# lucidrains/transfusion-pytorch

Measured on AMD Instinct MI355X. Metric: train samples/sec, dim512 d8 seq1024 text+latent, higher is better.
Workload: dtype bf16; 1 GPU; BASELINE config 2: Transfusion dim=512 depth=8 heads=8 dim_head=64 num_text_tokens=256 dim_latent=384; per-GPU batch 64 x seq 1024 (32 x [24 text tokens + (4,384) latent] per sample); step = pack + fwd + bwd + clip(0.5) + Adam(3e-4) (one GPU: no gradient exchange); global_batch=64, seq_len=1024, parallelism=dp1

## Files before the change

include/tfx.h:

```cpp
#ifndef TFX_H
#define TFX_H
#include <stdint.h>
#ifdef __cplusplus
extern "C" {
#endif

#ifndef TFX_BF16_DEFINED
typedef uint16_t tfx_bf16;
#endif

enum { TFX_EPI_BF16 = 0, TFX_EPI_F32 = 1, TFX_EPI_SILU = 2, TFX_EPI_RESID = 3, TFX_EPI_GEGLU = 4, TFX_EPI_GEGLU_BWD = 5, TFX_EPI_QKV_NORM_ROPE = 6 };

typedef struct {
  const tfx_bf16* A; int32_t lda;
  const tfx_bf16* A2; int32_t lda2; int32_t K1;
  const tfx_bf16* B; int32_t ldb;
  int32_t M, N, K;
  int32_t epi;
  void* C; int32_t ldc;
  void* C2; int32_t ldc2;
  const float* bias;
  const tfx_bf16* R; int32_t ldr; int32_t resid_mapped;
  const int32_t* rowmap;
  const int32_t* a_rowmap;
// ... 163 lines not shown
int tfx_attnres_finish(const tfx_attnres_src* src_dev, int32_t n, int32_t d, void* stream);
int tfx_adaln_pre_post_bwd(const tfx_adaln_pre_args* pre, const tfx_adaln_post_args* post, void* stream);

typedef struct {
  int32_t T, d;
  const tfx_bf16* x; tfx_bf16* y; const float* gamma;
  const tfx_bf16* dy; tfx_bf16* dx; float* dgamma;
} tfx_rmsnorm_args;
int tfx_rmsnorm_fwd(const tfx_rmsnorm_args* a, void* stream);
int tfx_rmsnorm_bwd(const tfx_rmsnorm_args* a, void* stream);

typedef struct {
  int32_t T, d;
  const int32_t* text_ids; const int32_t* tok_inst;
  const tfx_bf16* table;
  tfx_bf16* x;
  const tfx_bf16* dx; float* dtable;
} tfx_embed_args;
int tfx_embed_fwd(const tfx_embed_args* a, void* stream);
int tfx_embed_bwd(const tfx_embed_args* a, void* stream);

typedef struct {
  int32_t R, dl;
  const float* x; const float* eps;
  const int32_t* row_inst; const float* inst_time;
  tfx_bf16* xt; int32_t ld_xt;
  float* flow;
} tfx_noise_mix_args;
int tfx_noise_mix(const tfx_noise_mix_args* a, void* stream);

typedef struct { int32_t I, half; const float* times; const float* w; tfx_bf16* out; int32_t ld; } tfx_fourier_args;
int tfx_fourier(const tfx_fourier_args* a, void* stream);

typedef struct {
  int32_t T, V; const float* logits; int32_t ld;
  const int32_t* labels;
  float grad_scale;
  tfx_bf16* dlogits; int32_t ld_d;
  float* acc;
} tfx_ce_args;
int tfx_ce_fwd_bwd(const tfx_ce_args* a, void* stream);

typedef struct {
  int32_t R, dl; const float* pred; int32_t ld_pred; const float* flow;
  float grad_scale;
  tfx_bf16* dpred; int32_t ld_d;
  float* acc;
  int32_t accumulate;
  const int32_t* row_inst; const float* inst_time; float clean_eps;
  const float* recon_w; const int32_t* recon_inst; const float* recon_time; int32_t recon_mode;
} tfx_mse_args;
int tfx_mse_fwd_bwd(const tfx_mse_args* a, void* stream);
typedef struct {
  int32_t T, d; const tfx_bf16* pred; int32_t ld_pred; const tfx_bf16* target; int32_t ld_target;
  int32_t n_pad, n_valid;
  float grad_scale;
  tfx_bf16* dpred; int32_t ld_d;
  float* acc;
} tfx_cosine_args;
int tfx_cosine_fwd_bwd(const tfx_cosine_args* a, void* stream);
int tfx_output_to_flow(float* pred, const float* x, const float* eps, const int32_t* row_inst, const float* inst_time,
                       int32_t R, int32_t dl, float clean_eps, void* stream);

int tfx_sample_tokens(const float* logits, int32_t ld, int32_t B, int32_t V, float temperature, float min_p, const float* uniforms,
                      const int32_t* active, int32_t* out_ids, void* stream);
int tfx_sample_tokens_range(const float* logits, int32_t ld, int32_t B, int32_t V, int32_t V_draw, float temperature, float min_p, const float* uniforms,
                            const int32_t* active, int32_t* out_ids, void* stream);
int tfx_ode_axpy(const float* y, const float* f_cond, const float* f_uncond, float cfg_scale, float a, float* out, int64_t n, void* stream);
int tfx_ode_stage(const float* y, const float* ym, const float* ctl, int32_t B, int32_t Lc, int32_t dmax, float* x, int32_t H, int32_t Lq, int32_t dl,
                  const int32_t* rows0, void* stream);
int tfx_ode_update(float* y, float* ym, const float* ctl, int32_t B, int32_t Lc, int32_t dmax, const float* pred, int32_t H, int32_t Lq, int32_t dl,
                   float cfg_scale, const float* sel, const int32_t* rows0, void* stream);
enum { TFX_ODE_MAX_STAGES = 4 };
int tfx_ode_rk_axpy(const float* y, const float* k, int64_t k_stride, int32_t nk, float w0, float w1, float w2, float w3, const float* f_cond,
                    const float* f_uncond, float cfg_scale, float* k_out, float* out, int64_t n, void* stream);
int tfx_ode_rk_stage(const float* y, const float* k, const float* ctl, int32_t B, int32_t Lc, int32_t dmax, float* x, int32_t H, int32_t Lq, int32_t dl,
                     const int32_t* rows0, void* stream);
int tfx_ode_rk_update(float* y, float* k, const float* ctl, int32_t B, int32_t Lc, int32_t dmax, const float* pred, int32_t H, int32_t Lq, int32_t dl,
                      float cfg_scale, const float* sel, const int32_t* rows0, void* stream);

typedef struct { const float* src; int32_t ld_src, Rs, Cs; const int32_t* rowmap; tfx_bf16* dst; int32_t ld_dst, Rd, Cd; } tfx_cast_args;
int tfx_cast_rows(const tfx_cast_args* a, void* stream);
int tfx_cast_rows_t(const tfx_cast_args* a, void* stream);
typedef struct { const float* src; int32_t ld_src, Rs, Cs; const int32_t* rowmap; tfx_bf16* dst; int32_t ld_dst, Rd, Cd; int32_t transposed, first_block; } tfx_cast_job;
int tfx_cast_batch(const tfx_cast_job* jobs_dev, int32_t n_jobs, int32_t n_blocks, void* stream);
int tfx_gather_f32(const float* src, const int32_t* map, float* dst, int32_t n, void* stream);
int tfx_onehot_bf16(const int32_t* ids, const int32_t* tok_inst, tfx_bf16* out, int32_t T, int32_t ld, void* stream);
int tfx_scatter_rows_bf16(const tfx_bf16* src, int32_t ld_src, int32_t cols, tfx_bf16* dst, int32_t ld_dst, const int32_t* rowmap, int32_t R, void* stream);
int tfx_f32_to_bf16(const float* src, tfx_bf16* dst, int64_t n, void* stream);
int tfx_cast_block_bf16(const float* src, int32_t ld_src, tfx_bf16* dst, int32_t ld_dst, int32_t R, int32_t C, void* stream);
int tfx_silu_bwd(const tfx_bf16* dy, const tfx_bf16* pre, tfx_bf16* dx, int64_t n, void* stream);
int tfx_colsum_bf16(const tfx_bf16* src, int32_t ld, int32_t R, int32_t C, const int32_t* colmap, const int32_t* rowmap, float* out, void* stream);
int tfx_colsum_f32(const float* src, int32_t ld, int32_t R, int32_t C, float* out, void* stream);
int tfx_add_bf16(const tfx_bf16* a, const tfx_bf16* b, tfx_bf16* out, int64_t n, void* stream);
int tfx_scale_bf16_dev(tfx_bf16* x, int64_t n, const float* scale, void* stream);
int tfx_scale_bf16_copy(const tfx_bf16* src, tfx_bf16* dst, int64_t n, float scale, void* stream);

int tfx_sumsq(const float* g, int64_t n, float* sumsq, void* stream);
typedef struct {
  float* p; const float* g; float* m; float* v; int64_t n;
  float lr, beta1, beta2, eps, weight_decay, max_norm, grad_scale;
  int32_t step; const float* sumsq;
  const int64_t* skip; int32_t nskip;
} tfx_adam_args;
int tfx_adam_step(const tfx_adam_args* a, void* stream);

enum { TFX_ADAM_MAX_GROUPS = 8 };
typedef struct {
  float* p; const float* g; float* m; float* v; int64_t n;
  float lr, beta1, beta2, eps, weight_decay, max_norm, grad_scale;
  int32_t step; const float* sumsq;
  const int64_t* skip; int32_t nskip;
  int32_t decoupled;
  const int64_t* ranges; int32_t nrange, ngroup;
  float group_lr[TFX_ADAM_MAX_GROUPS], group_beta1[TFX_ADAM_MAX_GROUPS], group_beta2[TFX_ADAM_MAX_GROUPS], group_eps[TFX_ADAM_MAX_GROUPS],
        group_weight_decay[TFX_ADAM_MAX_GROUPS];
  int32_t group_decoupled[TFX_ADAM_MAX_GROUPS];
} tfx_adam_group_args;
int tfx_adam_step_groups(const tfx_adam_group_args* a, void* stream);

enum { TFX_SUMSQ_DET_PARTIALS = 1024 };
int tfx_sumsq_det(const float* g, int64_t n, float* partials, float* sumsq, void* stream);
int tfx_muon_plan(int32_t rows, int32_t cols, int32_t* flip, int32_t* m, int32_t* n, int32_t* m_pad, int32_t* n_pad, int32_t* gram_tiles,
                  int32_t* update_tiles, int32_t* prep_blocks);
int tfx_muon_step_launches(int32_t ns_steps, int32_t nmat);
typedef struct {
  int64_t off;
  int64_t s_off, t_off;
  int32_t rows, cols, ld_s, ld_t;
  int32_t blk0;
  float lr_ratio;
} tfx_muon_mat;
typedef struct {
  const tfx_muon_mat* mats; const int32_t* blk_mat; int32_t nmat, nblk;
  const float* g; float* buf; tfx_bf16* ws; float* partials;
  const float* sumsq; float max_norm, grad_scale, momentum; int32_t nesterov;
} tfx_muon_prep_args;
int tfx_muon_prep(const tfx_muon_prep_args* a, void* stream);
int tfx_muon_norm(const tfx_muon_mat* mats, int32_t nmat, const float* partials, float eps, float* inv, void* stream);
typedef struct {
  const tfx_bf16* P; const tfx_bf16* Q; const tfx_bf16* Z; tfx_bf16* C; tfx_bf16* Ct;
  const float* scale_z; const float* scale_acc;
  int32_t M, N, K, ldp, ldq, ldz, ldc, ldct;
  int32_t tile0;
  int32_t reserved;
} tfx_muon_gemm_problem;
int tfx_muon_gemm(const tfx_muon_gemm_problem* table, const int32_t* tile_prob, int32_t ntiles, float alpha, float beta, void* stream);
typedef struct {
  const tfx_muon_mat* mats; const int32_t* blk_mat; int32_t nmat, nblk;
  float* p; const tfx_bf16* ws; float lr, decay;
} tfx_muon_apply_args;
int tfx_muon_apply(const tfx_muon_apply_args* a, void* stream);
int tfx_ema_update(float* ema, const float* online, int64_t n, float decay, void* stream);

int tfx_allreduce_unique_id(void* out128);
int tfx_allreduce_init(int32_t rank, int32_t world, const void* unique_id128);
int tfx_allreduce_run(float* buf, int64_t count, void* stream);
int tfx_allreduce_destroy(void);

typedef struct { const void *p0, *p1, *p2, *p3, *p4; int64_t i0, i1, i2, i3; float f0; int32_t reserved; } tfx_raw_args;
enum { TFX_OP_GEMM_NT = 0, TFX_OP_GEMM_TN = 1, TFX_OP_ATTN_FWD = 2, TFX_OP_ATTN_BWD = 3, TFX_OP_ADALN_PRE_FWD = 4, TFX_OP_ADALN_PRE_BWD = 5,
       TFX_OP_ADALN_POST_FWD = 6, TFX_OP_ADALN_POST_BWD = 7, TFX_OP_QK_NORM_ROPE_FWD = 8, TFX_OP_QK_NORM_ROPE_BWD = 9, TFX_OP_ATTNRES_FWD = 10,
       TFX_OP_ATTNRES_BWD = 11, TFX_OP_RMSNORM_FWD = 12, TFX_OP_RMSNORM_BWD = 13, TFX_OP_EMBED_FWD = 14, TFX_OP_EMBED_BWD = 15,
       TFX_OP_NOISE_MIX = 16, TFX_OP_FOURIER = 17, TFX_OP_CE_FWD_BWD = 18, TFX_OP_MSE_FWD_BWD = 19, TFX_OP_CAST_ROWS = 20, TFX_OP_CAST_ROWS_T = 21,
       TFX_OP_ADAM_STEP = 22, TFX_OP_DECODE_ATTN = 23, TFX_OP_LASER_V_FWD = 24, TFX_OP_LASER_V_BWD = 25, TFX_OP_COSINE_FWD_BWD = 26,
       TFX_OP_OUTPUT_TO_FLOW = 32, TFX_OP_GATHER_F32 = 33, TFX_OP_ONEHOT_BF16 = 34, TFX_OP_SCATTER_ROWS_BF16 = 35, TFX_OP_F32_TO_BF16 = 36,
       TFX_OP_SILU_BWD = 37, TFX_OP_COLSUM_BF16 = 38, TFX_OP_COLSUM_F32 = 39, TFX_OP_ADD_BF16 = 40, TFX_OP_SCALE_BF16_DEV = 41, TFX_OP_CAST_BLOCK_BF16 = 42, TFX_OP_SCALE_BF16_COPY = 43, TFX_OP_ADALN_POST_PRE_FWD = 44, TFX_OP_LAYER_END_FWD = 45,
       TFX_OP_ATTNRES_PREP = 46, TFX_OP_ATTNRES_PULL_BWD = 47, TFX_OP_ATTNRES_FINISH = 52, TFX_OP_ADALN_PRE_POST_BWD = 53,
       TFX_OP_FORK = 48, TFX_OP_JOIN = 49, TFX_OP_JOIN_RECORD = 50, TFX_OP_JOIN_WAIT = 51 };
typedef struct { int32_t op; int32_t stream; const void* args; } tfx_launch;
int tfx_run_list(const tfx_launch* list, int32_t n, void* stream, int32_t* failed_at);
int tfx_graph_create(const tfx_launch* list, int32_t n, void** graph_out);
int tfx_graph_create_single(const tfx_launch* list, int32_t n, void** graph_out);
int tfx_graph_launch(void* graph, void* stream);
int tfx_graph_destroy(void* graph);
int tfx_list_fingerprint(const tfx_launch* list, int32_t n, int64_t* out);
int tfx_set_single_stream(int32_t on);

const char* tfx_version(void);

#ifdef __cplusplus
}
#endif
#endif
```

transfusion_pytorch_amd/csrc/runner.hip:

```cpp
#include <atomic>
#include <hip/hip_runtime.h>
#include <cstdlib>
#include <cstdint>
#include "../../include/tfx.h"

namespace {

inline int run_one(const tfx_launch& l, void* s) {
  const void* a = l.args;
  const tfx_raw_args* r = static_cast<const tfx_raw_args*>(a);
  switch (l.op) {
    case TFX_OP_GEMM_NT:          return tfx_gemm_nt(static_cast<const tfx_gemm_nt_args*>(a), s);
    case TFX_OP_GEMM_TN:          return tfx_gemm_tn(static_cast<const tfx_gemm_tn_args*>(a), s);
    case TFX_OP_ATTN_FWD:         return tfx_attn_fwd(static_cast<const tfx_attn_args*>(a), s);
    case TFX_OP_ATTN_BWD:         return tfx_attn_bwd(static_cast<const tfx_attn_args*>(a), s);
    case TFX_OP_ADALN_PRE_FWD:    return tfx_adaln_pre_fwd(static_cast<const tfx_adaln_pre_args*>(a), s);
    case TFX_OP_ADALN_PRE_BWD:    return tfx_adaln_pre_bwd(static_cast<const tfx_adaln_pre_args*>(a), s);
    case TFX_OP_ADALN_POST_FWD:   return tfx_adaln_post_fwd(static_cast<const tfx_adaln_post_args*>(a), s);
    case TFX_OP_ADALN_POST_BWD:   return tfx_adaln_post_bwd(static_cast<const tfx_adaln_post_args*>(a), s);
    case TFX_OP_QK_NORM_ROPE_FWD: return tfx_qk_norm_rope_fwd(static_cast<const tfx_qk_norm_rope_args*>(a), s);
    case TFX_OP_QK_NORM_ROPE_BWD: return tfx_qk_norm_rope_bwd(static_cast<const tfx_qk_norm_rope_args*>(a), s);
    case TFX_OP_ATTNRES_FWD:      return tfx_attnres_fwd(static_cast<const tfx_attnres_args*>(a), s);
    case TFX_OP_ATTNRES_BWD:      return tfx_attnres_bwd(static_cast<const tfx_attnres_args*>(a), s);
    case TFX_OP_RMSNORM_FWD:      return tfx_rmsnorm_fwd(static_cast<const tfx_rmsnorm_args*>(a), s);
    case TFX_OP_RMSNORM_BWD:      return tfx_rmsnorm_bwd(static_cast<const tfx_rmsnorm_args*>(a), s);
    case TFX_OP_EMBED_FWD:        return tfx_embed_fwd(static_cast<const tfx_embed_args*>(a), s);
    case TFX_OP_EMBED_BWD:        return tfx_embed_bwd(static_cast<const tfx_embed_args*>(a), s);
    case TFX_OP_NOISE_MIX:        return tfx_noise_mix(static_cast<const tfx_noise_mix_args*>(a), s);
    case TFX_OP_FOURIER:          return tfx_fourier(static_cast<const tfx_fourier_args*>(a), s);
    case TFX_OP_CE_FWD_BWD:       return tfx_ce_fwd_bwd(static_cast<const tfx_ce_args*>(a), s);
    case TFX_OP_MSE_FWD_BWD:      return tfx_mse_fwd_bwd(static_cast<const tfx_mse_args*>(a), s);
    case TFX_OP_CAST_ROWS:        return tfx_cast_rows(static_cast<const tfx_cast_args*>(a), s);
    case TFX_OP_CAST_ROWS_T:      return tfx_cast_rows_t(static_cast<const tfx_cast_args*>(a), s);
    case TFX_OP_ADAM_STEP:        return tfx_adam_step(static_cast<const tfx_adam_args*>(a), s);
    case TFX_OP_DECODE_ATTN:      return tfx_decode_attn(static_cast<const tfx_attn_args*>(a), s);
    case TFX_OP_LASER_V_FWD:      return tfx_laser_v_fwd(static_cast<const tfx_laser_v_args*>(a), s);
    case TFX_OP_LASER_V_BWD:      return tfx_laser_v_bwd(static_cast<const tfx_laser_v_args*>(a), s);
    case TFX_OP_COSINE_FWD_BWD:   return tfx_cosine_fwd_bwd(static_cast<const tfx_cosine_args*>(a), s);
    case TFX_OP_OUTPUT_TO_FLOW:
      return tfx_output_to_flow((float*)r->p0, (const float*)r->p1, (const float*)r->p2, (const int32_t*)r->p3, (const float*)r->p4,
                                (int32_t)r->i0, (int32_t)r->i1, r->f0, s);
    case TFX_OP_GATHER_F32:
      return tfx_gather_f32((const float*)r->p0, (const int32_t*)r->p1, (float*)r->p2, (int32_t)r->i0, s);
    case TFX_OP_ONEHOT_BF16:
      return tfx_onehot_bf16((const int32_t*)r->p0, (const int32_t*)r->p1, (tfx_bf16*)r->p2, (int32_t)r->i0, (int32_t)r->i1, s);
    case TFX_OP_SCATTER_ROWS_BF16:
      return tfx_scatter_rows_bf16((const tfx_bf16*)r->p0, (int32_t)r->i0, (int32_t)r->i1, (tfx_bf16*)r->p1, (int32_t)r->i2,
                                   (const int32_t*)r->p2, (int32_t)r->i3, s);
    case TFX_OP_F32_TO_BF16:
      return tfx_f32_to_bf16((const float*)r->p0, (tfx_bf16*)r->p1, r->i0, s);
    case TFX_OP_SILU_BWD:
      return tfx_silu_bwd((const tfx_bf16*)r->p0, (const tfx_bf16*)r->p1, (tfx_bf16*)r->p2, r->i0, s);
    case TFX_OP_COLSUM_BF16:
      return tfx_colsum_bf16((const tfx_bf16*)r->p0, (int32_t)r->i0, (int32_t)r->i1, (int32_t)r->i2, (const int32_t*)r->p1,
                             (const int32_t*)r->p2, (float*)r->p3, s);
    case TFX_OP_COLSUM_F32:
      return tfx_colsum_f32((const float*)r->p0, (int32_t)r->i0, (int32_t)r->i1, (int32_t)r->i2, (float*)r->p1, s);
    case TFX_OP_ADD_BF16:
      return tfx_add_bf16((const tfx_bf16*)r->p0, (const tfx_bf16*)r->p1, (tfx_bf16*)r->p2, r->i0, s);
    case TFX_OP_ADALN_POST_PRE_FWD:
      return tfx_adaln_post_pre_fwd((const tfx_adaln_post_args*)r->p0, (const tfx_adaln_pre_args*)r->p1, s);
    case TFX_OP_LAYER_END_FWD:
      return tfx_layer_end_fwd((const tfx_adaln_post_args*)r->p0, (const tfx_attnres_args*)r->p1, (const tfx_adaln_pre_args*)r->p2, s);
    case TFX_OP_ATTNRES_PREP:
      return tfx_attnres_prep((const tfx_attnres_src*)r->p0, (int32_t)r->i0, (int32_t)r->i1, s);
    case TFX_OP_ATTNRES_FINISH:
      return tfx_attnres_finish((const tfx_attnres_src*)r->p0, (int32_t)r->i0, (int32_t)r->i1, s);
    case TFX_OP_ATTNRES_PULL_BWD:
      return tfx_attnres_pull_bwd((const tfx_attnres_pull_args*)r->p0, (const tfx_adaln_post_args*)r->p1, s);
    case TFX_OP_ADALN_PRE_POST_BWD:
      return tfx_adaln_pre_post_bwd((const tfx_adaln_pre_args*)r->p0, (const tfx_adaln_post_args*)r->p1, s);
    case TFX_OP_CAST_BLOCK_BF16:
      return tfx_cast_block_bf16((const float*)r->p0, (int32_t)r->i0, (tfx_bf16*)r->p1, (int32_t)r->i1, (int32_t)r->i2, (int32_t)r->i3, s);
    case TFX_OP_SCALE_BF16_COPY:
      return tfx_scale_bf16_copy((const tfx_bf16*)r->p0, (tfx_bf16*)r->p1, r->i0, r->f0, s);
    case TFX_OP_SCALE_BF16_DEV:
      return tfx_scale_bf16_dev((tfx_bf16*)r->p0, r->i0, (const float*)r->p1, s);
    default: return -100;
  }
}

struct SideStream {
  hipStream_t stream = nullptr;
  hipEvent_t fork_ev[64] = {}, join_ev[64] = {};
  int ensure() {
    if (stream) return 0;
    int lo = 0, hi = 0;
    (void)hipDeviceGetStreamPriorityRange(&lo, &hi);
    if (hipStreamCreateWithPriority(&stream, hipStreamNonBlocking, lo) != hipSuccess) return -110;
    for (int i = 0; i < 64; ++i)
      if (hipEventCreateWithFlags(&fork_ev[i], hipEventDisableTiming) != hipSuccess ||
          hipEventCreateWithFlags(&join_ev[i], hipEventDisableTiming) != hipSuccess) return -111;
    return 0;
  }
};
constexpr int kMaxDevices = 16;
SideStream g_sides[kMaxDevices];
std::atomic<bool> g_single_stream{false};
thread_local int t_force_single = 0;
inline bool single_stream() { return t_force_single > 0 || g_single_stream.load(std::memory_order_relaxed); }
inline SideStream* side_of_current_device() {
  int dev = 0;
  if (hipGetDevice(&dev) != hipSuccess || dev < 0 || dev >= kMaxDevices) return nullptr;
  return &g_sides[dev];
}

}

extern "C" int tfx_run_list(const tfx_launch* list, int32_t n, void* stream, int32_t* failed_at) {
  if (n < 0 || (n > 0 && !list)) return -1;
  hipStream_t main_s = (hipStream_t)stream;
  SideStream* sp = nullptr;
  auto side = [&](int& rc) -> SideStream* {
    if (!sp && !(sp = side_of_current_device())) { rc = -112; return nullptr; }
    rc = sp->ensure();
    return rc == 0 ? sp : nullptr;
  };
  for (int32_t i = 0; i < n; ++i) {
    const tfx_launch& l = list[i];
    int rc = 0;
    if (!l.args) rc = -2;
    else if (l.op >= TFX_OP_FORK && l.op <= TFX_OP_JOIN_WAIT) {
      if (l.stream < 0 || l.stream >= 64) rc = -3;
      else if (single_stream()) rc = 0;
      else if (SideStream* gs = side(rc)) {
        SideStream& g_side = *gs;
        if (l.op == TFX_OP_FORK) {
          rc = (int)hipEventRecord(g_side.fork_ev[l.stream], main_s);
          if (rc == 0) rc = (int)hipStreamWaitEvent(g_side.stream, g_side.fork_ev[l.stream], 0);
        } else {
          if (l.op != TFX_OP_JOIN_WAIT) rc = (int)hipEventRecord(g_side.join_ev[l.stream], g_side.stream);
          if (rc == 0 && l.op != TFX_OP_JOIN_RECORD) rc = (int)hipStreamWaitEvent(main_s, g_side.join_ev[l.stream], 0);
        }
      }
    } else if (l.stream == 1 && !single_stream()) {
      if (SideStream* gs = side(rc)) rc = run_one(l, (void*)gs->stream);
    } else if (l.stream == 1) {
      rc = run_one(l, stream);
    } else if (l.stream == 0) {
      rc = run_one(l, stream);
    } else rc = -3;
    if (rc != 0) { if (failed_at) *failed_at = i; return rc; }
  }
  return 0;
}

namespace {
hipStream_t g_capture_streams[kMaxDevices] = {};
}
extern "C" int tfx_graph_create(const tfx_launch* list, int32_t n, void** graph_out) {
  if (!graph_out || n <= 0 || !list) return -1;
  *graph_out = nullptr;
  int dev = 0;
  if (hipGetDevice(&dev) != hipSuccess || dev < 0 || dev >= kMaxDevices) return -112;
  hipStream_t& g_capture_stream = g_capture_streams[dev];
  if (!g_capture_stream && hipStreamCreateWithFlags(&g_capture_stream, hipStreamNonBlocking) != hipSuccess) return -120;
// ... 97 lines not shown
```

transfusion_pytorch_amd/csrc/tokenwise.hip:

```cpp
#include "tfx_kernels.h"
#include <map>
#include <mutex>
#include <utility>
#include <cstdlib>

namespace tfx {

constexpr int WAVES = 4;
constexpr int MAXB = 1024;

template <int NC> struct Row {
  float v[NC][8];
};

template <int NC> TFX_DEV void load_row(Row<NC>& r, const bf16* p, int d, int lane) {
#pragma unroll
  for (int i = 0; i < NC; i++) {
    int c = lane + 64 * i;
    if (c * 8 < d) {
      bf16x8 x = *(const bf16x8*)(p + c * 8);
#pragma unroll
      for (int e = 0; e < 8; e++) r.v[i][e] = bf2f(x[e]);
    } else {
#pragma unroll
// ... 1640 lines not shown
      int rs = p.rowmap ? p.rowmap[r] : r;
      if (rs >= 0 && rs < p.Rs) v = p.src[(size_t)rs * p.ld_src + c];
    }
    tile[j][tx] = v;
  }
  __syncthreads();
  for (int j = ty; j < 32; j += 8) {
    int c = c0 + j, r = r0 + tx;
    if (c < p.Rd && r < p.ld_dst) p.dst[(size_t)c * p.ld_dst + r] = f2bf(tile[tx][j]);
  }
}
__global__ __launch_bounds__(256) void cast_rows_k(tfx_cast_args p) { cast_rows_body(p, blockIdx.x); }
__global__ __launch_bounds__(256) void cast_rows_t_k(tfx_cast_args p) {
  __shared__ float tile[32][33];
  cast_rows_t_body(p, blockIdx.x, blockIdx.y, tile);
}
TFX_DEV void cast8_body(const tfx_cast_args& p, long long blk) {
  const long long i = (blk * 256 + threadIdx.x) * 8;
  if (i >= (long long)p.Rd * p.ld_dst) return;
  const int r = (int)(i / p.ld_dst), c = (int)(i % p.ld_dst);
  const int rs = p.rowmap ? p.rowmap[r] : r;
  const int cmax = min(p.Cs, p.Cd);
  bf16x8 o;
  if (rs >= 0 && rs < p.Rs) {
    const float* sp = p.src + (size_t)rs * p.ld_src + c;
    if (c + 8 <= cmax && (((uintptr_t)sp) & 15) == 0) {
      const f32x4 a = *(const f32x4*)sp, b = *(const f32x4*)(sp + 4);
#pragma unroll
      for (int e = 0; e < 4; e++) { o[e] = f2bf(a[e]); o[4 + e] = f2bf(b[e]); }
    } else {
#pragma unroll
      for (int e = 0; e < 8; e++) o[e] = f2bf(c + e < cmax ? sp[e] : 0.f);
    }
  } else {
#pragma unroll
    for (int e = 0; e < 8; e++) o[e] = f2bf(0.f);
  }
  *(bf16x8*)(p.dst + i) = o;
}
TFX_DEV void cast64_t_body(const tfx_cast_args& p, int bx, int by, float (*tile)[65]) {
  const int r0 = bx * 64, c0 = by * 64;
  {
    const int cq = threadIdx.x & 15, rr = threadIdx.x >> 4;
    const int c = c0 + 4 * cq;
    int rs[4];
#pragma unroll
    for (int k = 0; k < 4; k++) {
      const int r = r0 + rr + 16 * k;
      rs[k] = r < p.Cd ? (p.rowmap ? p.rowmap[r] : r) : -1;
      if (rs[k] >= p.Rs) rs[k] = -1;
    }
    f32x4 v[4];
#pragma unroll
    for (int k = 0; k < 4; k++) {
      const f32x4 z = {0.f, 0.f, 0.f, 0.f};
      v[k] = z;
      if (rs[k] >= 0 && c < p.Cs) {
        const float* sp = p.src + (size_t)rs[k] * p.ld_src + c;
        if (c + 4 <= p.Cs && (((uintptr_t)sp) & 15) == 0) v[k] = *(const f32x4*)sp;
        else {
#pragma unroll
          for (int e = 0; e < 4; e++) if (c + e < p.Cs) v[k][e] = sp[e];
        }
      }
    }
#pragma unroll
    for (int k = 0; k < 4; k++)
#pragma unroll
      for (int e = 0; e < 4; e++) tile[rr + 16 * k][4 * cq + e] = v[k][e];
  }
  __syncthreads();
#pragma unroll
  for (int k = 0; k < 2; k++) {
    const int q = threadIdx.x + 256 * k, row = q >> 3, ch = q & 7;
    const int c = c0 + row, r = r0 + 8 * ch;
    if (c < p.Rd && r < p.ld_dst) {
      bf16x8 o;
#pragma unroll
      for (int e = 0; e < 8; e++) o[e] = f2bf(tile[8 * ch + e][row]);
      *(bf16x8*)(p.dst + (size_t)c * p.ld_dst + r) = o;
    }
  }
}
__global__ __launch_bounds__(256) void cast_batch_k(const tfx_cast_job* jobs, int n_jobs) {
  __shared__ float tile[64][65];
  int lo = 0, hi = n_jobs - 1;
  while (lo < hi) { const int mid = (lo + hi + 1) >> 1; if (jobs[mid].first_block <= (int)blockIdx.x) lo = mid; else hi = mid - 1; }
  const tfx_cast_job j = jobs[lo];
  const tfx_cast_args p = {j.src, j.ld_src, j.Rs, j.Cs, j.rowmap, j.dst, j.ld_dst, j.Rd, j.Cd};
  const int lb = blockIdx.x - j.first_block;
  if (j.transposed) { const int tx = (p.ld_dst + 63) / 64; cast64_t_body(p, lb % tx, lb / tx, tile); }
  else cast8_body(p, lb);
}
__global__ void onehot_k(const int* ids, const int* tok_inst, bf16* out, int T, int ld) {
  const long long i = ((long long)blockIdx.x * blockDim.x + threadIdx.x) * 8;
  if (i >= (long long)T * ld) return;
  const int t = (int)(i / ld), c = (int)(i % ld);
  const int id = tok_inst[t] < 0 ? max(ids[t], 0) : -1;
  bf16x8 o;
#pragma unroll
  for (int e = 0; e < 8; e++) o[e] = f2bf(c + e == id ? 1.f : 0.f);
  *(bf16x8*)(out + i) = o;
}
__global__ void scatter_rows_k(const bf16* src, int ld_src, int cols, bf16* dst, int ld_dst, const int* rowmap, int R) {
  const long long i = (long long)blockIdx.x * blockDim.x + threadIdx.x;
  const int cpr = cols / 8;
  if (i >= (long long)R * cpr) return;
  const int r = (int)(i / cpr), c = (int)(i % cpr) * 8;
  const int ro = rowmap[r];
  if (ro >= 0) *(bf16x8*)(dst + (size_t)ro * ld_dst + c) = *(const bf16x8*)(src + (size_t)r * ld_src + c);
}
__global__ void gather_f32_k(const float* src, const int* map, float* dst, int n) {
  int i = blockIdx.x * blockDim.x + threadIdx.x;
  if (i < n) dst[i] = map[i] >= 0 ? src[map[i]] : 0.f;
}
__global__ void f32_to_bf16_k(const float* src, bf16* dst, long long n) {
  long long i = ((long long)blockIdx.x * blockDim.x + threadIdx.x) * 4;
  if (i + 3 < n) {
    f32x4 v = *(const f32x4*)(src + i);
    bf16x4 o; o[0] = f2bf(v[0]); o[1] = f2bf(v[1]); o[2] = f2bf(v[2]); o[3] = f2bf(v[3]);
    *(bf16x4*)(dst + i) = o;
  } else for (; i < n; i++) dst[i] = f2bf(src[i]);
}
__global__ void silu_bwd_k(const bf16* dy, const bf16* pre, bf16* dx, long long n) {
  long long i = (long long)blockIdx.x * blockDim.x + threadIdx.x;
  if (i >= n) return;
  float x = bf2f(pre[i]), s = sigmoidf_(x);
  dx[i] = f2bf(bf2f(dy[i]) * s * (1.f + x * (1.f - s)));
}
__global__ void add_bf16_k(const bf16* a, const bf16* b, bf16* o, long long n) {
  long long i = ((long long)blockIdx.x * blockDim.x + threadIdx.x) * 8;
  if (i + 7 < n) {
    bf16x8 x = *(const bf16x8*)(a + i), y = *(const bf16x8*)(b + i), r;
#pragma unroll
    for (int e = 0; e < 8; e++) r[e] = f2bf(bf2f(x[e]) + bf2f(y[e]));
    *(bf16x8*)(o + i) = r;
  } else for (; i < n; i++) o[i] = f2bf(bf2f(a[i]) + bf2f(b[i]));
}

__global__ void scale_bf16_dev_k(bf16* x, long long n, const float* scale) {
  const float sc = *scale;
  if (sc == 1.f) return;
  long long i = ((long long)blockIdx.x * blockDim.x + threadIdx.x) * 8;
  if (i + 7 < n) {
    bf16x8 v = *(const bf16x8*)(x + i);
#pragma unroll
    for (int e = 0; e < 8; e++) v[e] = f2bf(bf2f(v[e]) * sc);
    *(bf16x8*)(x + i) = v;
  } else for (; i < n; i++) x[i] = f2bf(bf2f(x[i]) * sc);
}

template <typename T> __global__ __launch_bounds__(256) void colsum_k(const T* src, int ld, int R, int C, const int* colmap, const int* rowmap, float* out, int rows_per_block) {
  __shared__ float s[4][64];
  const int cx = threadIdx.x & 63, ry = threadIdx.x >> 6;
  const int c = blockIdx.x * 64 + cx;
  const int rbeg = blockIdx.y * rows_per_block, rend = min(R, rbeg + rows_per_block);
  float a = 0.f;
  if (c < C) for (int r = rbeg + ry; r < rend; r += 4) a += (float)src[(size_t)(rowmap ? rowmap[r] : r) * ld + c];
  s[ry][cx] = a;
  __syncthreads();
  if (ry == 0 && c < C) {
    float v = s[0][cx] + s[1][cx] + s[2][cx] + s[3][cx];
    int co = colmap ? colmap[c] : c;
    if (co >= 0 && v != 0.f) atomicAdd(out + co, v);
  }
}

__global__ __launch_bounds__(512) void colsum8_k(const bf16* src, int ld, int R, int C, const int* colmap, const int* rowmap, float* out, int rows_per_block) {
  __shared__ float s[8][64][9];
  const int cx = threadIdx.x & 63, ry = threadIdx.x >> 6;
  const int c0 = (blockIdx.x * 64 + cx) * 8;
  const int rbeg = blockIdx.y * rows_per_block, rend = min(R, rbeg + rows_per_block);
  float a[8];
#pragma unroll
  for (int e = 0; e < 8; e++) a[e] = 0.f;
  if (c0 < C) {
    int r = rbeg + ry;
    for (; r + 56 < rend; r += 64) {
      bf16x8 v[8];
#pragma unroll
      for (int u = 0; u < 8; u++) v[u] = *(const bf16x8*)(src + (size_t)(rowmap ? rowmap[r + 8 * u] : r + 8 * u) * ld + c0);
#pragma unroll
      for (int u = 0; u < 8; u++)
#pragma unroll
        for (int e = 0; e < 8; e++) a[e] += bf2f(v[u][e]);
    }
    for (; r < rend; r += 8) {
      bf16x8 v = *(const bf16x8*)(src + (size_t)(rowmap ? rowmap[r] : r) * ld + c0);
#pragma unroll
      for (int e = 0; e < 8; e++) a[e] += bf2f(v[e]);
    }
  }
#pragma unroll
  for (int e = 0; e < 8; e++) s[ry][cx][e] = a[e];
  __syncthreads();
  {
    const int cc = threadIdx.x >> 3, e = threadIdx.x & 7;
    const int col = (blockIdx.x * 64 + cc) * 8 + e;
    if (col < C) {
      float v = 0.f;
#pragma unroll
      for (int y = 0; y < 8; y++) v += s[y][cc][e];
      const int co = colmap ? colmap[col] : col;
      if (co >= 0 && v != 0.f) atomicAdd(out + co, v);
    }
  }
}

__global__ __launch_bounds__(256) void sumsq_k(const float* g, long long n, float* out) {
  __shared__ float sacc[WAVES];
  float s = 0.f;
  for (long long i = ((long long)blockIdx.x * blockDim.x + threadIdx.x) * 4; i < n; i += (long long)gridDim.x * blockDim.x * 4) {
    if (i + 3 < n) { f32x4 v = *(const f32x4*)(g + i); s += v[0] * v[0] + v[1] * v[1] + v[2] * v[2] + v[3] * v[3]; }
    else for (long long j = i; j < n; j++) s += g[j] * g[j];
  }
  s = wave_sum(s);
  if ((threadIdx.x & 63) == 0) sacc[threadIdx.x >> 6] = s;
  __syncthreads();
  if (threadIdx.x == 0) { float a = 0.f; for (int i = 0; i < WAVES; i++) a += sacc[i]; atomicAdd(out, a); }
}

__global__ __launch_bounds__(256) void adam_k(tfx_adam_args p, float step_size, float inv_sqrt_bc2) {
  const long long i = ((long long)blockIdx.x * blockDim.x + threadIdx.x) * 4;
  if (i >= p.n) return;
  if (p.nskip > 0) {
    int lo = 0, hi = p.nskip;
    while (lo < hi) { const int mid = (lo + hi) >> 1; if (p.skip[2 * mid + 1] > i) hi = mid; else lo = mid + 1; }
    if (lo < p.nskip && p.skip[2 * lo] <= i) return;
  }
  float coef = p.grad_scale;
  if (p.max_norm > 0.f) {
    float norm = sqrtf(p.sumsq[0]) * p.grad_scale;
    coef *= fminf(1.f, p.max_norm / (norm + 1e-6f));
  }
  if (i + 4 <= p.n) {
    const f32x4 g4 = *(const f32x4*)(p.g + i), w4 = *(const f32x4*)(p.p + i);
    f32x4 m4 = *(const f32x4*)(p.m + i), v4 = *(const f32x4*)(p.v + i), o4;
#pragma unroll
    for (int e = 0; e < 4; e++) {
      float g = g4[e] * coef;
      if (p.weight_decay != 0.f) g += p.weight_decay * w4[e];
      m4[e] = p.beta1 * m4[e] + (1.f - p.beta1) * g;
      v4[e] = p.beta2 * v4[e] + (1.f - p.beta2) * g * g;
      o4[e] = w4[e] - step_size * m4[e] / (sqrtf(v4[e]) * inv_sqrt_bc2 + p.eps);
    }
    *(f32x4*)(p.m + i) = m4; *(f32x4*)(p.v + i) = v4; *(f32x4*)(p.p + i) = o4;
  } else {
// ... 263 lines not shown
int tfx_attnres_finish(const tfx_attnres_src* src, int32_t n, int32_t d, void* s) {
  if (n <= 0) return 0;
  hipLaunchKernelGGL(attnres_finish_k, dim3((d + 255) / 256, n), dim3(256), 0, ST(s), src, d); RET();
}
int tfx_attnres_pull_bwd(const tfx_attnres_pull_args* a, const tfx_adaln_post_args* b, void* s) {
  if (!a || a->n_src < 1 || a->n_src > PULL_MAX_SRC || (a->d & 7) || a->d > 2048) return -2;
  if (b && (b->T != a->T || b->d != a->d || (const void*)b->g != (const void*)a->dh)) return -3;
  tfx_adaln_post_args none = {};
  const tfx_adaln_post_args& bb = b ? *b : none;
  const int hp = b ? 1 : 0;
  const size_t acc = (size_t)a->n_src * a->d * sizeof(float);
  const bool small = a->d <= 512 && a->n_src <= 8 && !a->k1;
  if (!small) {
    if (a->d > 1024) return -6;
    if (!a->k1 || a->ld_k1 < a->n_src) return -5;
    return a->d <= 512 ? pull_dma<1, 0>(*a, bb, hp, ST(s)) : pull_dma<2, 0>(*a, bb, hp, ST(s));
  }
  if (small) {
    auto fn = (b && b->dbias) ? attnres_pull_reg_k<1, 8, true> : attnres_pull_reg_k<1, 8, false>;
    const int items = a->n_seg > 0 ? a->n_seg : a->T;
    int grid = (items + 7) / 8; const int cap = resident_blocks(fn, 512, acc);
    if (grid > cap) grid = cap; if (grid < 1) grid = 1;
    hipLaunchKernelGGL(fn, dim3(grid), dim3(512), acc, ST(s), *a, bb, hp); RET();
  }
  return -6;
}
int tfx_embed_fwd(const tfx_embed_args* a, void* s) { DISPATCH_NC(a->d, hipLaunchKernelGGL(embed_fwd_k<NC>, dim3(grid_tokens(a->T)), dim3(256), 0, ST(s), *a)); RET(); }
int tfx_embed_bwd(const tfx_embed_args* a, void* s) { DISPATCH_NC(a->d, hipLaunchKernelGGL(embed_bwd_k<NC>, dim3(grid_tokens(a->T)), dim3(256), 0, ST(s), *a)); RET(); }

int tfx_qk_norm_rope_fwd(const tfx_qk_norm_rope_args* a, void* s) {
  long long nthreads = (long long)a->T * (a->cache ? 3 : 2) * a->H * 8;
  if (nthreads >= (1ll << 31)) return -3;
  hipLaunchKernelGGL(qk_norm_rope_fwd_k, dim3((unsigned)((nthreads + 255) / 256)), dim3(256), 0, ST(s), *a); RET();
}
int tfx_qk_norm_rope_bwd(const tfx_qk_norm_rope_args* a, void* s) {
  long long nthreads = (long long)a->T * 2 * a->H * 8;
  if (nthreads >= (1ll << 31)) return -3;
  long long g = (nthreads + 1023) / 1024;
  const long long cap = 256;
  if (g > cap) g = cap;
  hipLaunchKernelGGL(qk_norm_rope_bwd_k, dim3((unsigned)g), dim3(1024), 0, ST(s), *a); RET();
}
int tfx_noise_mix(const tfx_noise_mix_args* a, void* s) {
  long long n = (long long)a->R * a->ld_xt; if (n == 0) return 0;
  hipLaunchKernelGGL(noise_mix_k, dim3((unsigned)((n + 255) / 256)), dim3(256), 0, ST(s), *a); RET();
}
int tfx_fourier(const tfx_fourier_args* a, void* s) { if (a->I == 0) return 0; hipLaunchKernelGGL(fourier_k, dim3(a->I), dim3(256), 0, ST(s), *a); RET(); }
int tfx_ce_fwd_bwd(const tfx_ce_args* a, void* s) {
  int g = grid_tokens(a->T); if (g > 1024) g = 1024;
  hipLaunchKernelGGL(ce_k, dim3(g), dim3(256), 0, ST(s), *a); RET();
}
int tfx_mse_fwd_bwd(const tfx_mse_args* a, void* s) {
  long long n = (long long)a->R * a->ld_d; if (n == 0) return 0;
  long long g = (n + 255) / 256; if (g > 2048) g = 2048;
  hipLaunchKernelGGL(mse_k, dim3((unsigned)g), dim3(256), 0, ST(s), *a); RET();
}
int tfx_cosine_fwd_bwd(const tfx_cosine_args* a, void* s) {
  if (!a || a->T < 0 || a->d <= 0 || a->d > 2048 || (a->d % 64) || (a->ld_pred % 8) || (a->ld_target % 8) || (a->ld_d % 8) || a->ld_pred < a->d || a->ld_target < a->d || a->ld_d < a->d) return -1;
  if (!a->pred || !a->target || !a->dpred || !a->acc || a->n_pad < 0 || a->n_valid < 0) return -2;
  if (a->T == 0) return 0;
  DISPATCH_NC(a->d, hipLaunchKernelGGL(cosine_k<NC>, dim3(grid_capped(a->T)), dim3(256), 0, ST(s), *a)); RET();
}
int tfx_cast_rows(const tfx_cast_args* a, void* s) {
  long long n = (long long)a->Rd * a->ld_dst; if (n == 0) return 0;
  hipLaunchKernelGGL(cast_rows_k, dim3((unsigned)((n + 255) / 256)), dim3(256), 0, ST(s), *a); RET();
}
int tfx_cast_rows_t(const tfx_cast_args* a, void* s) {
  hipLaunchKernelGGL(cast_rows_t_k, dim3((a->ld_dst + 31) / 32, (a->Rd + 31) / 32), dim3(256), 0, ST(s), *a); RET();
}
int tfx_cast_batch(const tfx_cast_job* jobs_dev, int32_t n_jobs, int32_t n_blocks, void* s) {
  if (n_jobs <= 0 || n_blocks <= 0) return 0;
  hipLaunchKernelGGL(cast_batch_k, dim3(n_blocks), dim3(256), 0, ST(s), jobs_dev, n_jobs); RET();
}
int tfx_onehot_bf16(const int32_t* ids, const int32_t* tok_inst, tfx_bf16* out, int32_t T, int32_t ld, void* s) {
  if (T == 0) return 0; if (ld % 8) return -1;
  long long n = (long long)T * ld / 8;
  hipLaunchKernelGGL(onehot_k, dim3((unsigned)((n + 255) / 256)), dim3(256), 0, ST(s), ids, tok_inst, out, T, ld); RET();
}
int tfx_scatter_rows_bf16(const tfx_bf16* src, int32_t ld_src, int32_t cols, tfx_bf16* dst, int32_t ld_dst, const int32_t* rowmap, int32_t R, void* s) {
  if (R == 0) return 0; if (cols % 8 || ld_src % 8 || ld_dst % 8) return -1;
  long long n = (long long)R * (cols / 8);
  hipLaunchKernelGGL(scatter_rows_k, dim3((unsigned)((n + 255) / 256)), dim3(256), 0, ST(s), src, ld_src, cols, dst, ld_dst, rowmap, R); RET();
}
int tfx_gather_f32(const float* src, const int32_t* map, float* dst, int32_t n, void* s) {
  if (n == 0) return 0; hipLaunchKernelGGL(gather_f32_k, dim3((n + 255) / 256), dim3(256), 0, ST(s), src, map, dst, n); RET();
}
int tfx_f32_to_bf16(const float* src, tfx_bf16* dst, int64_t n, void* s) {
  if (n == 0) return 0; hipLaunchKernelGGL(f32_to_bf16_k, dim3((unsigned)((n / 4 + 256) / 256)), dim3(256), 0, ST(s), src, dst, (long long)n); RET();
}
int tfx_silu_bwd(const tfx_bf16* dy, const tfx_bf16* pre, tfx_bf16* dx, int64_t n, void* s) {
  if (n == 0) return 0; hipLaunchKernelGGL(silu_bwd_k, dim3((unsigned)((n + 255) / 256)), dim3(256), 0, ST(s), dy, pre, dx, (long long)n); RET();
}
int tfx_add_bf16(const tfx_bf16* a, const tfx_bf16* b, tfx_bf16* o, int64_t n, void* s) {
  if (n == 0) return 0; hipLaunchKernelGGL(add_bf16_k, dim3((unsigned)((n / 8 + 256) / 256)), dim3(256), 0, ST(s), a, b, o, (long long)n); RET();
}
int tfx_scale_bf16_dev(tfx_bf16* x, int64_t n, const float* scale, void* s) {
  if (n == 0) return 0;
  if (!x || !scale) return -1;
  hipLaunchKernelGGL(scale_bf16_dev_k, dim3((unsigned)((n / 8 + 256) / 256)), dim3(256), 0, ST(s), x, (long long)n, scale); RET();
}
static inline int colsum_rows_per_block(int R) { int rpb = (R + 63) / 64; return rpb < 4 ? 4 : rpb; }
int tfx_colsum_bf16(const tfx_bf16* src, int32_t ld, int32_t R, int32_t C, const int32_t* colmap, const int32_t* rowmap, float* out, void* s) {
  if (R == 0 || C == 0) return 0;
  if (C % 8 == 0 && ld % 8 == 0) {
    const int gx = (C + 511) / 512;
    int gy = 768 / gx; if (gy < 1) gy = 1;
    int rpb8 = (R + gy - 1) / gy; if (rpb8 < 64) rpb8 = 64;
    hipLaunchKernelGGL(colsum8_k, dim3(gx, (R + rpb8 - 1) / rpb8), dim3(512), 0, ST(s), src, ld, R, C, colmap, rowmap, out, rpb8); RET();
  }
  int rpb = colsum_rows_per_block(R);
  hipLaunchKernelGGL(colsum_k<bf16>, dim3((C + 63) / 64, (R + rpb - 1) / rpb), dim3(256), 0, ST(s), src, ld, R, C, colmap, rowmap, out, rpb); RET();
}
int tfx_colsum_f32(const float* src, int32_t ld, int32_t R, int32_t C, float* out, void* s) {
  if (R == 0 || C == 0) return 0;
  int rpb = colsum_rows_per_block(R);
  hipLaunchKernelGGL(colsum_k<float>, dim3((C + 63) / 64, (R + rpb - 1) / rpb), dim3(256), 0, ST(s), src, ld, R, C, (const int*)nullptr, (const int*)nullptr, out, rpb); RET();
}
int tfx_sumsq(const float* g, int64_t n, float* out, void* s) {
  if (n == 0) return 0;
  long long blocks = (n / 4 + 255) / 256; if (blocks > 2048) blocks = 2048; if (blocks < 1) blocks = 1;
  hipLaunchKernelGGL(sumsq_k, dim3((unsigned)blocks), dim3(256), 0, ST(s), g, (long long)n, out); RET();
}
int tfx_adam_step(const tfx_adam_args* a, void* s) {
  if (a->n == 0) return 0;
  if (((uintptr_t)a->p | (uintptr_t)a->g | (uintptr_t)a->m | (uintptr_t)a->v) & 15) return -1;
  if (a->nskip < 0 || (a->nskip > 0 && !a->skip)) return -1;
  const double bc1 = 1.0 - pow((double)a->beta1, (double)a->step), bc2 = 1.0 - pow((double)a->beta2, (double)a->step);
  const long long nthr = (a->n + 3) / 4;
  hipLaunchKernelGGL(adam_k, dim3((unsigned)((nthr + 255) / 256)), dim3(256), 0, ST(s), *a, (float)(a->lr / bc1), (float)(1.0 / sqrt(bc2))); RET();
}
int tfx_adam_step_groups(const tfx_adam_group_args* a, void* s) {
  if (a->nrange == 0 && a->decoupled == 0) {
    tfx_adam_args b;
    b.p = a->p; b.g = a->g; b.m = a->m; b.v = a->v; b.n = a->n; b.lr = a->lr; b.beta1 = a->beta1; b.beta2 = a->beta2; b.eps = a->eps;
    b.weight_decay = a->weight_decay; b.max_norm = a->max_norm; b.grad_scale = a->grad_scale; b.step = a->step; b.sumsq = a->sumsq;
    b.skip = a->skip; b.nskip = a->nskip;
    return tfx_adam_step(&b, s);
  }
  if (a->n == 0) return 0;
  if (a->n < 0 || (((uintptr_t)a->p | (uintptr_t)a->g | (uintptr_t)a->m | (uintptr_t)a->v) & 15)) return -1;
  if (a->nskip < 0 || (a->nskip > 0 && !a->skip)) return -1;
  if (a->nrange < 0 || (a->nrange > 0 && (!a->ranges || a->ngroup < 1 || a->ngroup > TFX_ADAM_MAX_GROUPS))) return -1;
  if (a->max_norm > 0.f && !a->sumsq) return -1;
  adam_consts c;
  for (int g = 0; g < TFX_ADAM_MAX_GROUPS; g++) {
    const int k = a->nrange > 0 && g < a->ngroup ? g : 0;
    const bool tab = a->nrange > 0;
    const float lr = tab ? a->group_lr[k] : a->lr, b1 = tab ? a->group_beta1[k] : a->beta1, b2 = tab ? a->group_beta2[k] : a->beta2;
    const float wd = tab ? a->group_weight_decay[k] : a->weight_decay;
    const bool dec = (tab ? a->group_decoupled[k] : a->decoupled) != 0;
    const double bc1 = 1.0 - pow((double)b1, (double)a->step), bc2 = 1.0 - pow((double)b2, (double)a->step);
    c.step_size[g] = (float)(lr / bc1); c.inv_sqrt_bc2[g] = (float)(1.0 / sqrt(bc2));
    c.beta1[g] = b1; c.beta2[g] = b2; c.eps[g] = tab ? a->group_eps[k] : a->eps;
    c.l2[g] = dec ? 0.f : wd;
    c.keep[g] = dec ? (float)(1.0 - (double)lr * (double)wd) : 1.f;
  }
  const long long nthr = (a->n + 3) / 4;
  hipLaunchKernelGGL(adam_groups_k, dim3((unsigned)((nthr + 255) / 256)), dim3(256), 0, ST(s), *a, c); RET();
}
int tfx_output_to_flow(float* pred, const float* x, const float* eps, const int32_t* row_inst, const float* inst_time,
                       int32_t R, int32_t dl, float clean_eps, void* s) {
  if (R <= 0 || dl <= 0) return 0;
  if ((long long)R * dl >= (1ll << 31)) return -1;
  hipLaunchKernelGGL(output_to_flow_k, dim3((unsigned)(((long long)R * dl + 255) / 256)), dim3(256), 0, ST(s), pred, x, eps, row_inst, inst_time, R, dl, clean_eps); RET();
}
int tfx_ema_update(float* ema, const float* online, int64_t n, float decay, void* s) {
  if (n <= 0) return 0;
  if (((uintptr_t)ema | (uintptr_t)online) & 15) return -1;
  hipLaunchKernelGGL(ema_k, dim3((unsigned)(((n + 3) / 4 + 255) / 256)), dim3(256), 0, ST(s), ema, online, (long long)n, decay); RET();
}
int tfx_gemm_nt(const tfx_gemm_nt_args* a, void* s) { return gemm_nt(*a, ST(s)); }
int tfx_gemm_tn(const tfx_gemm_tn_args* a, void* s) { return gemm_tn(*a, ST(s)); }
int tfx_gemm_nt_plan(const tfx_gemm_nt_args* a, int32_t* kind, int32_t* grid) { return gemm_nt_plan(*a, kind, grid); }
int tfx_gemm_tn_plan(const tfx_gemm_tn_args* a, int32_t* kind, int32_t* tiles, int32_t* splits, int32_t* grid) { return gemm_tn_plan(*a, kind, tiles, splits, grid); }
int tfx_attn_fwd(const tfx_attn_args* a, void* s) { return attn_fwd(*a, ST(s)); }
int tfx_attn_bwd(const tfx_attn_args* a, void* s) { return attn_bwd(*a, ST(s)); }
int tfx_mfma_peak_probe(const void* ops, float* out, int32_t iters, int32_t blocks, void* s) {
  if (!ops || !out || iters <= 0 || blocks <= 0) return -1;
  hipLaunchKernelGGL(mfma_peak_k, dim3(blocks), dim3(256), 0, ST(s), (const bf16x8*)ops, out, iters); RET();
}
int tfx_laser_v_fwd(const tfx_laser_v_args* a, void* s) {
  if (!a || a->T < 0 || a->H <= 0 || !(a->c > 0.f)) return -1;
  if (a->T == 0) return 0;
  if (!a->v || !a->vl || ((a->ld_v | a->ld_vl) & 7) || a->ld_v < a->H * 64 || a->ld_vl < a->H * 64 || (((uintptr_t)a->v | (uintptr_t)a->vl) & 15)) return -2;
  const long long nch = (long long)a->T * a->H * 8;
  if (nch >= (1ll << 31)) return -4;
  hipLaunchKernelGGL(laser_v_fwd_k, dim3((unsigned)((nch + 255) / 256)), dim3(256), 0, ST(s), *a, (unsigned)nch); RET();
}
int tfx_laser_v_bwd(const tfx_laser_v_args* a, void* s) {
  if (!a || a->T < 0 || a->H <= 0 || !(a->c > 0.f)) return -1;
  if (a->T == 0) return 0;
  if (!a->v || !a->dvl || !a->dv || ((a->ld_v | a->ld_dvl | a->ld_dv) & 7) || a->ld_v < a->H * 64 || a->ld_dvl < a->H * 64 || a->ld_dv < a->H * 64 ||
      (((uintptr_t)a->v | (uintptr_t)a->dvl | (uintptr_t)a->dv) & 15)) return -2;
  const long long nch = (long long)a->T * a->H * 8;
  if (nch >= (1ll << 31)) return -4;
  hipLaunchKernelGGL(laser_v_bwd_k, dim3((unsigned)((nch + 255) / 256)), dim3(256), 0, ST(s), *a, (unsigned)nch); RET();
}
const char* tfx_version(void) { return "tfx-hip gfx950 r5-laser-muon-selfflow-adamgroups-oderk"; }

// ... 2 lines not shown
```

transfusion_pytorch_amd/engine.py:

```python
from __future__ import annotations

import ctypes
import os
import weakref

import torch

from . import capi
from .params import ModelDims, ParamStore, pad_to

BF16 = torch.bfloat16
E = capi.ENUMS


def _p(t, *idx):
    for i in idx:
        t = t[i]
    return t.data_ptr()


def skip_sources(md: ModelDims):
    stack, src = [], {}
    for i in range(md.depth):
        layer = i + 1
# ... 140 lines not shown
        assert not units or (cache is not None and tile_attn), 'compacted plans are decode plans on the tiled attention kernel (the row ranges are its arguments)'
        self.cache = cache
        self.tile_attn = tile_attn
        assert cache is None or not training
        self.dp_groups = dp_groups
        self.bwd_cuts = []
        self.ps, self.md, self.b, self.n, self.I, self.R = ps, md, b, n, I, dict(R)
        self.T = T = b * n
        dev = ps.device
        d, hd, D, dip, ldq, nt3 = md.dim, md.hdk, md.depth, md.dip, md.ldq, md.nt3
        self.nbytes = 0
        def z(*s, dtype=BF16):
            t = torch.zeros(*s, device=dev, dtype=dtype); self.nbytes += t.numel() * t.element_size(); return t
        def e(*s, dtype=BF16):
            t = torch.empty(*s, device=dev, dtype=dtype); self.nbytes += t.numel() * t.element_size(); return t
        I1 = max(I, 1)
        self.idx = z(7, max(T, 1, 4 * units[0] if units else 1), dtype=torch.int32)
        self.text_ids, self.cache_pos, self.kv_end, self.rot_pos, self.tok_inst, self.q_start, self.labels = (self.idx[r, :T] if r != 1 else self.idx[r] for r in range(7))
        if units:
            U = units[0]
            self.unit_row0, self.unit_cnt, self.unit_blk0, self.unit_txt = (self.idx[6, k * U:(k + 1) * U] for k in range(4))
        self.inst_time = z(I1, dtype=torch.float32)
        self.row_tok = {t: z(r, dtype=torch.int32) for t, r in R.items()}
        self.rowbuf = None
        if cache is not None and R and len(set(R.values())) == 1:
            r = next(iter(R.values()))
            self.row_stride = rs = (r + 3) // 4 * 4
            self.rowbuf = z(2 * len(R) * rs + ctl_rows * max(b, units[0] if units else 0), dtype=torch.int32)
            self.row_tok = {t: self.rowbuf[k * rs:k * rs + r] for k, t in enumerate(R)}
            self.ctl = self.rowbuf[2 * len(R) * rs:].view(torch.float32)
        self.row_inst = {t: z(r, dtype=torch.int32) for t, r in R.items()}
        self.row_gat = {t: z(r, dtype=torch.int32) for t, r in R.items()} if (training and cache is None) else self.row_tok
        self._rows_dep = {t: [] for t in R}
        self.hid = e(D + 1, T, d)
        self.xres = [self.hid[0]] + [e(T, d) for _ in range(D)]
        nl = D if training else 1
        nkv = D if (training or cache is None) else 1
        self._li = (lambda i: i) if training else (lambda i: 0)
        self._lkv = (lambda i: i) if nkv == D else (lambda i: 0)
        xa_shared = None if training else e(T, d)
        self.xa = {i: (e(T, d) if training else xa_shared) for i in range(D) if md.has_skip(i)}
        self.stats = e(4, nl, T, dtype=torch.float32)
        self.ua = e(nl, T, d); self.uf = e(nl, T, d)
        self.qkvg = z(nkv, T, ldq); self.qkr = e(nkv, T, 2 * hd); self.og = z(nl, T, hd) if units else e(nl, T, hd)
        self.lse = e(nl, units[0], md.heads, units[1], dtype=torch.float32) if units else e(nl, b, md.heads, n, dtype=torch.float32)
        self.ya = e(nl, T, d); self.xb = e(nl, T, d); self.yf = e(nl, T, d)
        self.ag = e(nl, T, 2 * dip); self.hm = e(nl, T, dip)
        self.embed = e(T, d)
        self.logits = e(T, md.vp, dtype=torch.float32); self.dlogits = e(T, md.vp)
        self.fe = z(I1, md.kf); self.cond = e(I1, 4 * d); self.pre = e(I1, 4 * d)
        self.tables = z(I1, nt3, dtype=torch.float32)
        self.lat = {}
        self.ext, self.ext_add = set(md.ext_types) & set(R), set(md.pos_types) & set(R)
        for t, r in R.items():
            dl = md.dim_latents[t]; dlp = pad_to(dl, 64)
            if t in self.ext:
                self.lat[t] = dict(tok=z(r, d), gemb=z(r, d))
                continue
            self.lat[t] = dict(x=e(r, dl, dtype=torch.float32), eps=z(r, dl, dtype=torch.float32), xt=z(r, dlp),
                               flow=e(r, dl, dtype=torch.float32), pred=e(r, dl, dtype=torch.float32), dpred=z(r, dlp))
        for t in self.ext_add:
            self.lat[t]['add'] = z(R[t], d)
        self.acc = z(max(8, 2 + 3 * len(md.dim_latents)), dtype=torch.float32)
        self.tap0, self.taps, self._tap_buf = None, {}, {}
        self.vel = LaunchList()
        self.rec = LaunchList()
        self.cos_tab = self.sin_tab = None
        self.sc_plan = z(D, 8, dtype=torch.float32)
        self.vl = self.vlc = None
        if md.laser:
            if cache is None:
                self.vl = e(nl, T, hd)
            else:
                side = ps.__dict__.setdefault('_laser_side', weakref.WeakValueDictionary())
                key = (cache.data_ptr(), tuple(cache.shape), tuple(cache.stride()))
                self.vlc = side.get(key)
                if self.vlc is None:
                    self.vlc = e(D, cache.shape[1] * cache.shape[2], hd)
                    side[key] = self.vlc
        self.fwd, self.bwd = LaunchList(), LaunchList()
        self.noise_args = {}
        self.loaded_structure = None
        self._seg_args = []
        self.seg_start = z(max(T, 1), dtype=torch.int32); self.seg_len = z(max(T, 1), dtype=torch.int32)
        self.pull = training and D <= 32 and md.dim <= 1024
        if self.pull:
            self.arsave = [e(T, i + 2, 4, dtype=torch.float32) for i in range(D)]
            self.arerr = e(D, T, d)
        self._build_forward()
        if training:
            self.dH = e(D + 1, T, d)
            self.gx = {i: e(T, d) for i in range(D) if md.has_skip(i)}; self.du = e(T, d)
            env = os.environ.get('TFX_SIDE_STREAM')
            self.side = D <= 30 and (env == '1' or (env is None and md.dim <= 1024))
            nb = 2 if self.side else 1
            self.dy_f = [e(T, d) for _ in range(nb)]; self.dy_a = [e(T, d) for _ in range(nb)] if self.side else self.dy_f
            self.dskip = {j: e(T, d) for j in set(skip_sources(md).values())}
            self.dqkvg_p = [z(T, ldq) for _ in range(nb)]; self.dog = e(T, hd); self.do_eff = e(T, hd)
            self.dqk = e(T, 2 * hd) if os.environ.get('TFX_ATTN_QKNR', '1') == '0' else None
            self.delta = e(b, md.heads, n, dtype=torch.float32)
            self.dag_p = [e(T, 2 * dip) for _ in range(nb)]; self.dembed = e(T, d); self.gfin = e(T, d); self.dx0 = e(T, d)
            self.dtables = z(I1, nt3, dtype=torch.float32); self.dtab_bf = e(I1, nt3)
            self.dcond = e(I1, 4 * d); self.dpre = e(I1, 4 * d)
            self.onehot = e(T, md.vp)
            self._build_backward()

    def _nt(self, lst, algo_n=None, algo_k=None, **kw):
        a = capi.make_args('tfx_gemm_nt_args', **kw)
        a._algo_flops = 2.0 * kw['M'] * (algo_n or kw['N']) * (algo_k or kw['K'])
        lst.append(('tfx_gemm_nt', a))

    def _tn(self, lst, M, N, K, **kw):
        splits = 0
        kw.setdefault('k_valid', K)
        algo_n = kw.pop('algo_n', None)
        side = kw.pop('side', False)
        a = capi.make_args('tfx_gemm_tn_args', M=M, N=N, K=K, splits=splits, accumulate=1, alpha=1.0, **kw)
        a._algo_flops = 2.0 * M * (algo_n or N) * kw['k_valid']
        lst.append(Side(('tfx_gemm_tn', a)) if side else ('tfx_gemm_tn', a))

    def _tn_group(self, lst, M, problems, side=False):
        if len(problems) < 2 or os.environ.get('TFX_TN_GROUP', '1') == '0':
            for (N, K, kw) in problems:
                self._tn(lst, M, N, K, side=side, **kw)
            return
        structs, flops = [], 0.0
        for (N, K, kw) in problems:
            kw = dict(kw); kw.setdefault('k_valid', K)
            algo_n = kw.pop('algo_n', None)
            a = capi.make_args('tfx_gemm_tn_args', M=M, N=N, K=K, splits=0, accumulate=1, alpha=1.0, **kw)
            flops += 2.0 * M * (algo_n or N) * kw['k_valid']
            structs.append(a)
        for a, b in zip(structs, structs[1:]):
            a.group_next = ctypes.addressof(b)
        head = structs[0]
        head._chain = structs[1:]
        head._algo_flops = flops
        lst.append(Side(('tfx_gemm_tn', head)) if side else ('tfx_gemm_tn', head))

    def _k(self, lst, fn, struct, **kw):
        lst.append((fn, capi.make_args(struct, **kw)))

    def _raw(self, lst, fn, *args):
        lst.append((fn, args))

    def _hbm(self, lst, passes, extra_bytes=0):
        if lst.meta is None:
            lst.meta = {}
        lst.meta[len(lst) - 1] = ('hbm', passes * self.T * self.md.dim * 2 + extra_bytes)

    def _tab(self, i, w):
        off = ((i * 2 + w) * 3 * self.md.dim) * 4
        return self.tables.data_ptr() + off, (self.dtables.data_ptr() + off if hasattr(self, 'dtables') else 0)

    def _build_forward(self):
        ps, md, T, I = self.ps, self.md, self.T, self.I
        d, hd, D, dip, ldq, nt3, H = md.dim, md.hdk, md.depth, md.dip, md.ldq, md.nt3, md.heads
        S = ps.shadows
        L = self.fwd
        pp = ps.ptr
        if self.cache is not None:
            self.row_src = {t: torch.zeros(r, device=self.ps.device, dtype=torch.int32) for t, r in self.R.items()}
            if self.rowbuf is not None:
                r, M, rs = next(iter(self.R.values())), len(self.R), self.row_stride
                self.row_src = {t: self.rowbuf[(M + k) * rs:(M + k) * rs + r] for k, t in enumerate(self.R)}
        self._clean_launch, self.clean_mode = {}, ('model' if self.cache is not None else 'latent')
        for t, r in self.R.items():
            dl = md.dim_latents[t]; dlp = pad_to(dl, 64); lt = self.lat[t]
            if t in self.ext:
                self._raw(L, capi.lib().tfx_scatter_rows_bf16, lt['tok'].data_ptr(), d, d, self.hid[0].data_ptr(), d, self.row_tok[t].data_ptr(), r)
            else:
                self._k(L, 'tfx_noise_mix', 'tfx_noise_mix_args', R=r, dl=dl, x=lt['x'], eps=lt['eps'], row_inst=self.row_inst[t],
                        inst_time=self.inst_time, xt=lt['xt'], ld_xt=dlp, flow=lt['flow'])
                self.noise_args[t] = L[-1][1]
                if dl == d:
                    self._raw(L, capi.lib().tfx_scatter_rows_bf16, lt['xt'].data_ptr(), dlp, d, self.hid[0].data_ptr(), d, self.row_tok[t].data_ptr(), r)
                    lt['proj'] = lt['xt']
                elif md.model_output_clean:
                    lt['proj'] = torch.zeros(r, d, device=self.ps.device, dtype=BF16); self.nbytes += r * d * 2
                    self._nt(L, algo_k=dl, A=lt['xt'], lda=dlp, B=S[f'in{t}'], ldb=dlp, M=r, N=d, K=dlp, epi=E['TFX_EPI_BF16'], C=lt['proj'], ldc=d,
                             bias=pp(f'latent_to_model_projs.{t}.bias'))
                    self._raw(L, capi.lib().tfx_scatter_rows_bf16, lt['proj'].data_ptr(), d, d, self.hid[0].data_ptr(), d, self.row_tok[t].data_ptr(), r)
                else:
                    self._nt(L, algo_k=dl, A=lt['xt'], lda=dlp, B=S[f'in{t}'], ldb=dlp, M=r, N=d, K=dlp, epi=E['TFX_EPI_BF16'], C=self.hid[0], ldc=d,
                             bias=pp(f'latent_to_model_projs.{t}.bias'), rowmap=self.row_tok[t])
            if md.model_output_clean and t not in self.ext:
                self._clean_q(L, t, r)
            if t in self.ext_add:
                self._nt(L, A=lt['add'], lda=d, B=S['eye'], ldb=d, M=r, N=d, K=d, epi=E['TFX_EPI_RESID'], C=self.hid[0], ldc=d,
                         R=self.hid[0], ldr=d, resid_mapped=1, rowmap=self.row_tok[t])
        self._k(L, 'tfx_embed_fwd', 'tfx_embed_args', T=T, d=d, text_ids=self.text_ids, tok_inst=self.tok_inst, table=S['embed'], x=self.hid[0])
        self._hbm(L, 1)
        self.fwd_cond = (len(L), len(L))
        if I > 0:
            self._k(L, 'tfx_fourier', 'tfx_fourier_args', I=I, half=d // 2, times=self.inst_time, w=ps.fourier_w, out=self.fe, ld=md.kf)
            self._nt(L, algo_k=d + 1, A=self.fe, lda=md.kf, B=S['time'], ldb=md.kf, M=I, N=4 * d, K=md.kf, epi=E['TFX_EPI_SILU'], C=self.cond, ldc=4 * d,
                     C2=self.pre, ldc2=4 * d, bias=pp('transformer.to_time_cond.1.bias'))
            self._nt(L, A=self.cond, lda=4 * d, B=S['ada'], ldb=4 * d, M=I, N=nt3, K=4 * d, epi=E['TFX_EPI_F32'], C=self.tables, ldc=nt3,
                     bias=pp('transformer.layers.0.1.to_film.bias'))
            self.fwd_cond = (self.fwd_cond[0], len(L))
        src = skip_sources(md)
        fused_pre = {}
# ... 139 lines not shown
        ck = dict(cache=self.cache[i], ld_cache=2 * hd, cache_pos=self.cache_pos) if self.cache is not None else {}
        self._k(L, 'tfx_qk_norm_rope_fwd', 'tfx_qk_norm_rope_args', T=T, H=H, qkv=self.qkvg[lkv], ld_qkv=ldq, qk=self.qkr[lkv], ld_qk=2 * hd,
                gamma_q=gam('q'), gamma_k=gam('k'), rot_pos=self.rot_pos,
                cos_tab=0, sin_tab=0, q_scale=md.dim_head ** -0.5, norm_scale=md.dim_head ** 0.5, **ck, **plan_kw)
        self._rope_args = getattr(self, '_rope_args', []) + [L[-1][1]]
        L.meta = L.meta or {}
        L.meta[len(L) - 1] = ('hbm', 2 * 2 * T * hd * 2)
        self._laser_fwd(L, i)
        self._k(L, 'tfx_attn_fwd' if (self.cache is None or self.tile_attn) else 'tfx_decode_attn', 'tfx_attn_args', **self._attn_kw(i))

    def _laser_fwd(self, L, i):
        md, hd = self.md, self.md.hdk
        if not md.laser:
            return
        if self.cache is None:
            self._k(L, 'tfx_laser_v_fwd', 'tfx_laser_v_args', T=self.T, H=md.heads, v=_p(self.qkvg, self._lkv(i)) + 2 * 2 * hd, ld_v=md.ldq,
                    vl=self.vl[self._li(i)], ld_vl=hd, c=md.laser)
            rows = self.T
        else:
            ck = self.cache[i]
            rows = int(ck.shape[0]) * int(ck.shape[1])
            self._k(L, 'tfx_laser_v_fwd', 'tfx_laser_v_args', T=rows, H=md.heads, v=ck.data_ptr() + 2 * hd, ld_v=2 * hd,
                    vl=self.vlc[i], ld_vl=hd, c=md.laser)
        L.meta = L.meta or {}
        L.meta[len(L) - 1] = ('hbm', 2 * rows * hd * 2)

    def _clean_q(self, L, t, r):
        md, d = self.md, self.md.dim
        dl = md.dim_latents[t]; lt = self.lat[t]
        lt['q'] = torch.empty(r, dl, device=self.ps.device, dtype=torch.float32)
        self._nt(L, A=lt['proj'], lda=lt['proj'].shape[1], B=self.ps.shadows[f'outp{t}'], ldb=d, M=r, N=dl, K=d, epi=E['TFX_EPI_F32'], C=lt['q'], ldc=dl)

    def _clean_flow(self, L, t, r):
        md = self.md
        dl = md.dim_latents[t]; lt = self.lat[t]
        self._clean_launch[t] = [lt['pred'].data_ptr(), lt['q'].data_ptr() if self.clean_mode == 'model' else lt['x'].data_ptr(), None,
                                 self.row_inst[t].data_ptr(), self.inst_time.data_ptr(), r, dl, float(md.clean_eps)]
        L.append((capi.lib().tfx_output_to_flow, self._clean_launch[t]))

    def set_clean_mode(self, mode: str):
        assert mode in ('latent', 'model')
        self.clean_mode = mode
        for t, a in self._clean_launch.items():
            lt = self.lat[t]
            a[1] = lt['q'].data_ptr() if mode == 'model' else lt['x'].data_ptr()
            a[2] = None if mode == 'model' else self.noise_args[t].eps

    def _attn_kw(self, i, bwd=False):
        md, hd, ldq = self.md, self.md.hdk, self.md.ldq
        li, lkv = self._li(i), self._lkv(i)
        kw = dict(q=self.qkr[lkv], k=_p(self.qkr, lkv) + 2 * hd, v=_p(self.qkvg, lkv) + 2 * 2 * hd, ld_q=2 * hd, ld_k=2 * hd, ld_v=ldq,
                  gate=_p(self.qkvg, lkv) + 2 * 3 * hd, ld_gate=ldq, kv_end=self.kv_end, q_start=self.q_start, out=self.og[li], ld_out=hd,
                  lse=self.lse[li], b=self.units[0] if self.units else self.b, h=md.heads, n=self.units[1] if self.units else self.n, softcap=50.0)
        if self.units:
            kw.update(q_row0=self.unit_row0, q_cnt=self.unit_cnt)
        if self.sc_plan is not None:
            kw['sc_plan'] = self.sc_plan[i]
        if self.cache is not None:
            ck = self.cache[i]
            kw.update(k=ck.data_ptr(), v=ck.data_ptr() + 2 * hd, ld_k=2 * hd, ld_v=2 * hd, n_kv=int(ck.shape[1]))
        if md.laser:
            kw.update(v=self.vl[li] if self.cache is None else self.vlc[i], ld_v=hd, laser=1)
        if bwd:
            dqkvg = self.dqkvg_p[i % len(self.dqkvg_p)]
            kw.update(dout=self.dog, ld_dout=hd, do_eff=self.do_eff, ld_do=hd, delta=self.delta,
                      dgate=dqkvg.data_ptr() + 2 * 3 * hd, ld_dgate=ldq, dq=self.dqk if self.dqk is not None else 0,
                      dk=self.dqk.data_ptr() + 2 * hd if self.dqk is not None else 0,
                      dv=dqkvg.data_ptr() + 2 * 2 * hd, ld_dq=2 * hd, ld_dk=2 * hd, ld_dv=ldq)
        return kw

    def set_rope_tables(self, cos_tab, sin_tab):
        if self.cos_tab is not None and (self.cos_tab.data_ptr() != cos_tab.data_ptr() or self.sin_tab.data_ptr() != sin_tab.data_ptr()):
            self.fwd.invalidate_graphs()
        self.cos_tab, self.sin_tab = cos_tab, sin_tab
        for a in getattr(self, '_rope_args', []):
            a.cos_tab, a.sin_tab = cos_tab.data_ptr(), sin_tab.data_ptr()
        for a in getattr(self, '_rope_nt_args', []):
            a.qk_cos, a.qk_sin = cos_tab.data_ptr(), sin_tab.data_ptr()
        for a in getattr(self, '_rope_attn_args', []):
            a.nr_cos, a.nr_sin = cos_tab.data_ptr(), sin_tab.data_ptr()

    def set_segments(self, seg_start, seg_len):
        n_seg = int(seg_start.numel())
        self.seg_start[:n_seg].copy_(seg_start); self.seg_len[:n_seg].copy_(seg_len)
        for a in self._seg_args:
            a.n_seg = n_seg

    def set_rows(self, R_true: dict):
        for t, r in R_true.items():
            assert r <= self.R[t]
            for obj, key in [(self.noise_args.get(t), 'R'), (getattr(self, '_mse_args', {}).get(t), 'R'), (getattr(self, '_vel_args', {}).get(t), 'R'),
                             (getattr(self, '_rec_args', {}).get(t), 'R'), *self._rows_dep[t]]:
                if obj is None:
                    continue
                if isinstance(obj, list):
                    obj[key] = r
                else:
                    setattr(obj, key, r)
            lt = self.lat[t]
            if r < self.R[t] and 'xt' in lt:
                lt['xt'][r:].zero_()
                if 'dpred' in lt:
                    lt['dpred'][r:].zero_()
            if self.row_gat is not self.row_tok:
                torch.clamp(self.row_tok[t], min=0, out=self.row_gat[t])

    def load_structure(self, S, rope, tok_inst, kv_end, q_start, rot_pos, segments=None, rows=None, set_rows=False):
        self.set_rope_tables(*rope)
        self.tok_inst.copy_(tok_inst.view(-1)); self.kv_end.copy_(kv_end); self.q_start.copy_(q_start); self.rot_pos.copy_(rot_pos)
        if segments is not None:
            self.set_segments(*segments)
        if rows is not None:
            for t, cap in self.R.items():
                row_tok, row_inst = rows.get(t, (None, None))
                r = 0 if row_tok is None else int(row_tok.numel())
                if r < cap:
                    self.row_tok[t].fill_(-1); self.row_inst[t].zero_()
                if r:
                    self.row_tok[t][:r].copy_(row_tok); self.row_inst[t][:r].copy_(row_inst)
            if set_rows:
                self.set_rows({t: int(v[0].numel()) for t, v in rows.items()})
        self.loaded_structure = S

    def set_noise(self, t: int, eps_ptr):
        self.noise_args[t].eps = eps_ptr
        if t in getattr(self, '_clean_launch', {}) and self.clean_mode == 'latent':
            self._clean_launch[t][2] = eps_ptr

    def set_ce_vocab(self, V: int):
        self._ce_args.V = V

    def set_loss_scales(self, ce_scale: float, mse_scales: dict):
        self._ce_args.grad_scale = ce_scale
        for t, s in mse_scales.items():
            self._mse_args[t].grad_scale = s

    def _build_backward(self):
        ps, md, T, I = self.ps, self.md, self.T, self.I
        d, hd, D, di, dip, ldq, nt3, H = md.dim, md.hdk, md.depth, md.di, md.dip, md.ldq, md.nt3, md.heads
        S = ps.shadows
        L = self.bwd
        pp, gp = ps.ptr, ps.grad_ptr
        lib = capi.lib()
        gmap = ps._maps['geglu']
        self.clean_bwd = LaunchList()
        if md.model_output_clean:
            C = self.clean_bwd
            for t, r in self.R.items():
                if t in self.ext:
                    continue
                dl = md.dim_latents[t]; dlp = pad_to(dl, 64); lt = self.lat[t]
                lt['ndpred'] = torch.zeros(r, dlp, device=self.ps.device, dtype=BF16)
                self._raw(C, lib.tfx_scale_bf16_copy, lt['dpred'].data_ptr(), lt['ndpred'].data_ptr(), r * dlp, -1.0)
                self._tn(C, r, dl, d, A=lt['ndpred'], lda=dlp, a_cols=dlp, B=lt['proj'], ldb=lt['proj'].shape[1], b_cols=d,
                         C=gp(f'model_to_latent_projs.{t}.weight'), ldc=d)
                if dl != d:
                    lt['dpx'] = torch.empty(r, d, device=self.ps.device, dtype=BF16)
                    self._nt(C, algo_k=dl, A=lt['ndpred'], lda=dlp, B=S[f'outp_t{t}'], ldb=dlp, M=r, N=d, K=dlp, epi=E['TFX_EPI_BF16'], C=lt['dpx'], ldc=d)
                    self._tn(C, r, d, dl, A=lt['dpx'], lda=d, a_cols=d, B=lt['xt'], ldb=dlp, b_cols=dlp, C=gp(f'latent_to_model_projs.{t}.weight'), ldc=dl)
                    self._raw(C, lib.tfx_colsum_bf16, lt['dpx'].data_ptr(), d, r, d, None, None, gp(f'latent_to_model_projs.{t}.bias'))
        self._nt(L, algo_k=md.vocab, A=self.dlogits, lda=md.vp, B=S['logits_t'], ldb=md.vp, M=T, N=d, K=md.vp, epi=E['TFX_EPI_BF16'], C=self.dembed, ldc=d)
        self._tn(L, T, md.vocab, d, A=self.dlogits, lda=md.vp, a_cols=md.vp, B=self.embed, ldb=d, b_cols=d, C=gp('to_text_logits.weight'), ldc=d)
        for t, r in self.R.items():
            dl = md.dim_latents[t]; dlp = pad_to(dl, 64); lt = self.lat[t]
            if t in self.ext:
                self._nt(L, A=lt['gemb'], lda=d, B=S['eye'], ldb=d, M=r, N=d, K=d, epi=E['TFX_EPI_RESID'], C=self.dembed, ldc=d,
                         R=self.dembed, ldr=d, resid_mapped=1, rowmap=self.row_tok[t])
                continue
            self._nt(L, algo_k=dl, A=lt['dpred'], lda=dlp, B=S[f'outp_t{t}'], ldb=dlp, M=r, N=d, K=dlp, epi=E['TFX_EPI_RESID'], C=self.dembed, ldc=d,
                     R=self.dembed, ldr=d, resid_mapped=1, rowmap=self.row_tok[t])
            self._tn(L, r, dl, d, A=lt['dpred'], lda=dlp, a_cols=dlp, B=self.embed, ldb=d, b_cols=d, b_rowmap=self.row_gat[t],
                     C=gp(f'model_to_latent_projs.{t}.weight'), ldc=d)
        self.tap_final = len(L)
        self._k(L, 'tfx_rmsnorm_bwd', 'tfx_rmsnorm_args', T=T, d=d, x=self.xres[D], gamma=pp('transformer.norm.gamma'), dy=self.dembed,
                dx=self.gfin, dgamma=gp('transformer.norm.gamma'))
        self._hbm(L, 3)
        src = skip_sources(md)
        pushed = set(src.values())
        g = self.gfin
        side = self.side
        def sync(op, slot):
            if side:
                L.append((op, slot))
        pull = self.pull
        if pull:
            self.dsum = torch.empty(D, T, device=ps.device, dtype=torch.float32)
            self.wtab = torch.empty(2, D, d, device=ps.device, dtype=torch.float32)
            self.nbytes += self.dsum.numel() * 4 + self.wtab.numel() * 4
            SRC = capi.STRUCTS['tfx_attnres_src']
            recs = (SRC * D)()
            for j in range(D):
                pj = f'transformer.layers.{j}.3'
                gj = self.gfin if j == D - 1 else (self.gx[j + 1] if md.has_skip(j + 1) else self.dH[j + 2])
                for k, v in dict(g=gj, save=self.arsave[j], dsum=self.dsum[j], w=self.wtab[0, j], dw=self.wtab[1, j], gamma=pp(f'{pj}.norm_keys.gamma'),
                                 pq=pp(f'{pj}.pseudo_queries'), dgamma=gp(f'{pj}.norm_keys.gamma'), dpq=gp(f'{pj}.pseudo_queries'), L=j + 2).items():
                    setattr(recs[j], k, v.data_ptr() if hasattr(v, 'data_ptr') else v)
            raw = torch.frombuffer(bytearray(ctypes.string_at(ctypes.addressof(recs), ctypes.sizeof(recs))), dtype=torch.uint8)
            self._src_tab = raw.to(ps.device)
            self._src_size = ctypes.sizeof(SRC)
            self._raw(L, lib.tfx_attnres_prep, self._src_tab.data_ptr(), D, d)
        self._pull_args = {}
        def pull_launch(l, out_own, add, dh, post):
            j0 = max(l - 1, 0)
            ns = D - j0
            export = ns > 8 or d > 512
            if export and not hasattr(self, 'k1buf'):
                self.k1buf = torch.zeros(T, 32, device=ps.device, dtype=BF16); self.nbytes += self.k1buf.numel() * 2
            a = capi.make_args('tfx_attnres_pull_args', T=T, d=d, l=l, n_src=ns, h=self.hid[l], src=self._src_tab.data_ptr() + j0 * self._src_size,
                               out_own=out_own, out_err=self.arerr[l - 1] if out_own is not None else None, add=add, dh=dh,
                               seg_start=self.seg_start, seg_len=self.seg_len, n_seg=0, k1=self.k1buf if export else None, ld_k1=32)
            self._seg_args.append(a)
            self._pull_args[l] = a
            self._keep = getattr(self, '_keep', []) + [a, post]
            self._raw(L, lib.tfx_attnres_pull_bwd, ctypes.addressof(a), ctypes.addressof(post) if post is not None else None)
            self._hbm(L, ns + 6 if post is not None else ns + 4, 12 * ns * T)
            if export:
                self._tn(L, T, ns, d, A=self.k1buf, lda=32, a_cols=32, B=self.hid[l], ldb=d, b_cols=d, C=self.wtab[1, j0], ldc=d)
        for i in range(D - 1, -1, -1):
            p = f'transformer.layers.{i}'
            x_in = self.xres[i]
            x_a = self.xa[i] if md.has_skip(i) else x_in
            (ta, dta), (tf, dtf) = self._tab(i, 0), self._tab(i, 1)
            par = i % len(self.dag_p)
            dy_f, dy_a, dag, dqkvg = self.dy_f[par], self.dy_a[par], self.dag_p[par], self.dqkvg_p[par]
            if i + 2 <= D - 1:
                sync('tfx_join_wait', i + 2)
            G = self.dH[i + 1]
            a_postf = capi.make_args('tfx_adaln_post_args', T=T, d=d, y=self.yf[i], tok_inst=self.tok_inst, table=tf, ld_table=nt3,
                                     layerscale=pp(f'{p}.2.layerscale'), g=G, dy=dy_f, dtable=dtf, dlayerscale=gp(f'{p}.2.layerscale'),
                                     seg_start=self.seg_start, seg_len=self.seg_len, n_seg=0, dbias=gp(f'{p}.2.fn.net.3.bias'))
            self._seg_args.append(a_postf)
            if pull:
                pull_launch(i + 1, self.xres[i + 1], None, G, a_postf)
            else:
                g2 = self.dskip[i + 1] if (i + 1) in pushed else None
                self._k(L, 'tfx_attnres_bwd', 'tfx_attnres_args', T=T, d=d, L=i + 2, hiddens=self.hid, stride_h=T * d,
                        gamma=pp(f'{p}.3.norm_keys.gamma'), pq=pp(f'{p}.3.pseudo_queries'), g=g, g2=capi.ptr(g2), dhiddens=self.dH, stride_dh=T * d,
                        first=1 if i == D - 1 else 0, dgamma=gp(f'{p}.3.norm_keys.gamma'), dpq=gp(f'{p}.3.pseudo_queries'))
                L.append(('tfx_adaln_post_bwd', a_postf))
            self._nt(L, algo_n=di, A=dy_f, lda=d, B=S[f'ff2_t{i}'], ldb=d, M=T, N=dip, K=d, epi=E['TFX_EPI_GEGLU_BWD'], C=dag, ldc=2 * dip,
                     aux=self.ag[i], ldaux=2 * dip)
            sync('tfx_fork', 2 * i)
            ff_grp = [(d, di, dict(A=dy_f, lda=d, a_cols=d, B=self.hm[i], ldb=dip, b_cols=dip, C=gp(f'{p}.2.fn.net.3.weight'), ldc=di)),
                      (2 * dip, d, dict(algo_n=2 * di, A=dag, lda=2 * dip, a_cols=2 * dip, B=self.uf[i], ldb=d, b_cols=d, rowmap=gmap,
                                        C=gp(f'{p}.2.fn.net.0.weight'), ldc=d, colsum=gp(f'{p}.2.fn.net.0.bias')))]
            self._tn_group(L, T, ff_grp, side=side)
            self._nt(L, algo_k=2 * di, A=dag, lda=2 * dip, B=S[f'ff1_t{i}'], ldb=2 * dip, M=T, N=d, K=2 * dip, epi=E['TFX_EPI_BF16'], C=self.du, ldc=d)
            a_pref = capi.make_args('tfx_adaln_pre_args', T=T, d=d, x=self.xb[i], tok_inst=self.tok_inst, table=tf, ld_table=nt3,
                                    gamma_text=pp(f'{p}.2.layernorm_gamma'), mean=_p(self.stats, 2, i), rstd=_p(self.stats, 3, i), du=self.du, dx=G,
                                    dtable=dtf, dgamma_text=gp(f'{p}.2.layernorm_gamma'), seg_start=self.seg_start, seg_len=self.seg_len, n_seg=0)
            a_posta = capi.make_args('tfx_adaln_post_args', T=T, d=d, y=self.ya[i], tok_inst=self.tok_inst, table=ta, ld_table=nt3,
                                     layerscale=pp(f'{p}.1.layerscale'), g=G, dy=dy_a, dtable=dta, dlayerscale=gp(f'{p}.1.layerscale'),
                                     seg_start=self.seg_start, seg_len=self.seg_len, n_seg=0)
            self._seg_args += [a_pref, a_posta]
            self._keep = getattr(self, '_keep', []) + [a_pref, a_posta]
            self._raw(L, lib.tfx_adaln_pre_post_bwd, ctypes.addressof(a_pref), ctypes.addressof(a_posta))
            self._hbm(L, 6)
            self._nt(L, algo_n=md.hd, A=dy_a, lda=d, B=S[f'out_t{i}'], ldb=d, M=T, N=hd, K=d, epi=E['TFX_EPI_BF16'], C=self.dog, ldc=hd)
            gam = (lambda nm: S[f'g{nm}{i}']) if md.dim_head != 64 else (lambda nm: pp(f'{p}.1.fn.{nm}_norm.gamma'))
            if os.environ.get('TFX_ATTN_QKNR', '1') != '0':
                self._k(L, 'tfx_attn_bwd', 'tfx_attn_args', **self._attn_kw(i, bwd=True), nr_qkv=self.qkvg[i], nr_ld_qkv=ldq, nr_dqkv=dqkvg, nr_ld_dqkv=ldq,
                        nr_gamma_q=gam('q'), nr_gamma_k=gam('k'), nr_rot_pos=self.rot_pos, nr_cos=0, nr_sin=0, nr_q_scale=md.dim_head ** -0.5,
                        nr_norm_scale=md.dim_head ** 0.5, nr_dgamma_q=gp(f'{p}.1.fn.q_norm.gamma'), nr_dgamma_k=gp(f'{p}.1.fn.k_norm.gamma'))
                self._rope_attn_args = getattr(self, '_rope_attn_args', []) + [L[-1][1]]
            else:
                self._k(L, 'tfx_attn_bwd', 'tfx_attn_args', **self._attn_kw(i, bwd=True))
                self._k(L, 'tfx_qk_norm_rope_bwd', 'tfx_qk_norm_rope_args', T=T, H=H, qkv=self.qkvg[i], ld_qkv=ldq, gamma_q=gam('q'),
                        gamma_k=gam('k'), rot_pos=self.rot_pos, cos_tab=0, sin_tab=0, q_scale=md.dim_head ** -0.5, norm_scale=md.dim_head ** 0.5,
                        dqk=self.dqk, ld_dqk=2 * hd, dqkv=dqkvg, ld_dqkv=ldq, dgamma_q=gp(f'{p}.1.fn.q_norm.gamma'), dgamma_k=gp(f'{p}.1.fn.k_norm.gamma'))
                self._rope_args = getattr(self, '_rope_args', []) + [L[-1][1]]
                L.meta = L.meta or {}
                L.meta[len(L) - 1] = ('hbm', 3 * 2 * T * hd * 2)
            if md.laser:
                dv = dqkvg.data_ptr() + 2 * 2 * hd
                self._k(L, 'tfx_laser_v_bwd', 'tfx_laser_v_args', T=T, H=H, v=_p(self.qkvg, i) + 2 * 2 * hd, ld_v=ldq, c=md.laser,
                        dvl=dv, ld_dvl=ldq, dv=dv, ld_dv=ldq)
                L.meta = L.meta or {}
                L.meta[len(L) - 1] = ('hbm', 3 * T * hd * 2)
            self._nt(L, algo_k=md.nq, A=dqkvg, lda=ldq, B=S[f'qkvg_t{i}'], ldb=ldq, M=T, N=d, K=ldq, epi=E['TFX_EPI_BF16'], C=self.du, ldc=d)
            self._k(L, 'tfx_adaln_pre_bwd', 'tfx_adaln_pre_args', T=T, d=d, x=x_a, tok_inst=self.tok_inst, table=ta, ld_table=nt3,
                    gamma_text=pp(f'{p}.1.layernorm_gamma'), mean=_p(self.stats, 0, i), rstd=_p(self.stats, 1, i), du=self.du, dx=G,
                    dtable=dta, dgamma_text=gp(f'{p}.1.layernorm_gamma'), seg_start=self.seg_start, seg_len=self.seg_len, n_seg=0,
                    dx_add=self.dskip[i] if (pull and i in pushed) else None)
            self._hbm(L, 4 + (1 if (pull and i in pushed) else 0))
            self._seg_args.append(L[-1][1])
            sync('tfx_fork', 2 * i + 1)
            grp = [(d, hd, dict(A=dy_a, lda=d, a_cols=d, B=self.og[i], ldb=hd, b_cols=hd, C=gp(f'{p}.1.fn.to_out.1.weight'), ldc=md.hd,
                                k_group=0 if md.dim_head == 64 else md.dim_head)),
                   (md.nqk, d, dict(algo_n=md.nq, A=dqkvg, lda=ldq, a_cols=ldq, B=self.ua[i], ldb=d, b_cols=d, C=gp(f'{p}.1.fn.to_qk.0.weight'), ldc=d,
                                    rowmap=ps._maps['heads'] if md.dim_head != 64 else None))]
            if md.has_skip(i):
                sk = self.xres[src[i]]
                grp.append((d, d, dict(A=G, lda=d, a_cols=d, B=x_in, ldb=d, b_cols=d, C=gp(f'{p}.0.weight'), ldc=2 * d)))
                grp.append((d, d, dict(A=G, lda=d, a_cols=d, B=sk, ldb=d, b_cols=d, C=gp(f'{p}.0.weight', d), ldc=2 * d)))
            self._tn_group(L, T, grp, side=side)
            per = -(-D // self.dp_groups) if self.dp_groups > 0 else D
            if I > 0 and i % per == 0:
                hi = min(i + per, D)
                off, cols = i * 2 * 3 * d, (hi - i) * 2 * 3 * d
                w_item = lambda it: L.append(Side(it) if side else it)
                w_item((lib.tfx_cast_block_bf16, (self.dtables.data_ptr() + 4 * off, nt3, self.dtab_bf.data_ptr() + 2 * off, nt3, I, cols)))
                self._tn(L, I, cols, 4 * d, side=side, A=self.dtab_bf.data_ptr() + 2 * off, lda=nt3, a_cols=cols, B=self.cond, ldb=4 * d, b_cols=4 * d,
                         C=gp(f'{p}.1.to_film.weight'), ldc=4 * d)
                w_item((lib.tfx_colsum_f32, (self.dtables.data_ptr() + 4 * off, nt3, I, cols, gp(f'{p}.1.to_film.bias'))))
            sync('tfx_join_record', i)
            if self.dp_groups > 0:
                if i % per == 0:
                    sync('tfx_join_wait', i)
                    self.bwd_cuts.append((len(L), i, min(i + per, D) - 1))
            if md.has_skip(i):
                st = S[f'skip_t{i}']
                self._nt(L, A=G, lda=d, B=st, ldb=d, M=T, N=d, K=d, epi=E['TFX_EPI_RESID'], C=self.gx[i], ldc=d, R=G, ldr=d)
                self._nt(L, A=G, lda=d, B=st[d:], ldb=d, M=T, N=d, K=d, epi=E['TFX_EPI_BF16'], C=self.dskip[src[i]], ldc=d)
                g = self.gx[i]
            else:
                g = G
        sync('tfx_join', 63)
        if pull:
            pull_launch(0, None, g, self.dx0, None)
            self._raw(L, lib.tfx_attnres_finish, self._src_tab.data_ptr(), D, d)
        else:
            self._raw(L, lib.tfx_add_bf16, g.data_ptr(), self.dH[0].data_ptr(), self.dx0.data_ptr(), T * d)
            if 0 in pushed:
                self._raw(L, lib.tfx_add_bf16, self.dx0.data_ptr(), self.dskip[0].data_ptr(), self.dx0.data_ptr(), T * d)
        self._raw(L, lib.tfx_onehot_bf16, self.text_ids.data_ptr(), self.tok_inst.data_ptr(), self.onehot.data_ptr(), T, md.vp)
        self._x0_param_grads(L, self.dx0)
        if I > 0:
            self._nt(L, A=self.dtab_bf, lda=nt3, B=S['ada_t'], ldb=nt3, M=I, N=4 * d, K=nt3, epi=E['TFX_EPI_BF16'], C=self.dcond, ldc=4 * d)
            self._raw(L, lib.tfx_silu_bwd, self.dcond.data_ptr(), self.pre.data_ptr(), self.dpre.data_ptr(), I * 4 * d)
            self._tn(L, I, 4 * d, d + 1, A=self.dpre, lda=4 * d, a_cols=4 * d, B=self.fe, ldb=md.kf, b_cols=md.kf,
                     C=gp('transformer.to_time_cond.1.weight'), ldc=d + 1)
            self._raw(L, lib.tfx_colsum_bf16, self.dpre.data_ptr(), 4 * d, I, 4 * d, None, None, gp('transformer.to_time_cond.1.bias'))

    def _x0_param_grads(self, L, dx0):
        md, T, d = self.md, self.T, self.md.dim
        gp, lib = self.ps.grad_ptr, capi.lib()
        self._tn(L, T, md.vocab, d, A=self.onehot, lda=md.vp, a_cols=md.vp, B=dx0, ldb=d, b_cols=d, C=gp('text_embed.weight'), ldc=d)
        for t, r in self.R.items():
            dl = md.dim_latents[t]; dlp = pad_to(dl, 64); lt = self.lat[t]
            if dl == d or t in self.ext:
                continue
            self._tn(L, r, d, dl, A=dx0, lda=d, a_cols=d, a_rowmap=self.row_gat[t], B=lt['xt'], ldb=dlp, b_cols=dlp,
                     C=gp(f'latent_to_model_projs.{t}.weight'), ldc=dl)
            cs = [dx0.data_ptr(), d, int(self.noise_args[t].R), d, None, self.row_tok[t].data_ptr(), gp(f'latent_to_model_projs.{t}.bias')]
            self._rows_dep[t].append((cs, 2))
            L.append((lib.tfx_colsum_bf16, cs))

    def set_taps(self, grads: dict, n_true: int):
        D, d = self.md.depth, self.md.dim
        self.clear_taps()
        if not grads:
            return
        if not self.pull:
            raise NotImplementedError('hidden taps need the pull-form AttentionResidual backward (depth <= 32 and dim <= 1024): the push form has no '
                                      'place where a hidden\'s gradient is formed once')
        for k, g in grads.items():
            assert 0 <= k <= D + 1
            buf = self.tap_buffer(k)
            if n_true < self.n:
                buf[:, n_true:].zero_()
            if g.data_ptr() != buf.data_ptr():
                buf[:, :n_true].copy_(g)
            if k == 0:
                lo = self.tap_buffer('0 lo')
                lo.zero_()
                if g.dtype != BF16:
                    lo[:, :n_true].copy_(g.float() - buf[:, :n_true].float())
                if self.tap0 is None:
                    self.tap0 = LaunchList()
                    for src in (buf, lo):
                        self._x0_param_grads(self.tap0, src)
            self.taps[k] = buf
            if 1 <= k <= D:
                self._pull_args[k].add = buf.data_ptr()

    def tap_buffer(self, k):
        buf = self._tap_buf.get(k)
        if buf is None:
            buf = self._tap_buf[k] = torch.zeros(self.b, self.n, self.md.dim, device=self.ps.device, dtype=BF16); self.nbytes += buf.numel() * 2
        return buf

    def clear_taps(self):
        for k in self.taps:
            if 1 <= k <= self.md.depth:
                self._pull_args[k].add = None
        self.taps = {}

    def run_bwd(self, stream, lo=0, hi=None):
        hi = len(self.bwd) if hi is None else hi
        taps = self.taps
        pos = self.tap_final
        if self.md.depth + 1 in taps and lo <= pos < hi:
            Plan.run(self.bwd, stream, lo, pos, graph='auto')
            dst, buf = self.dembed, taps[self.md.depth + 1]
            capi.check(capi.lib().tfx_add_bf16(dst.data_ptr(), buf.data_ptr(), dst.data_ptr(), dst.numel(), ctypes.c_void_p(stream)), 'tfx_add_bf16')
            lo = pos
        Plan.run(self.bwd, stream, lo, hi, graph='auto')
        if 0 in taps and hi == len(self.bwd):
            Plan.run(self.tap0, stream)

    def tap0_rows(self, index):
        if 0 not in self.taps:
            return None
        d = self.md.dim
        return self.taps[0].view(-1, d).index_select(0, index).float() + self.tap_buffer('0 lo').view(-1, d).index_select(0, index).float()

    @staticmethod
    def run(launches, stream, lo=0, hi=None, graph=False):
        lib = capi.lib()
        sp = ctypes.c_void_p(stream)
        if isinstance(launches, LaunchList):
            n = len(launches)
            lo = max(0, lo if lo >= 0 else n + lo)
            hi = n if hi is None else min(n, hi if hi >= 0 else n + hi)
            if hi <= lo:
                return
            if graph == 'auto':
                if TRAIN_GRAPH and launches.replay_auto(lo, hi, sp):
                    return
            elif graph:
                rc = lib.tfx_graph_launch(ctypes.c_void_p(launches.graph(lo, hi)), sp)
                if rc != 0:
                    raise capi.TfxError(f'tfx_graph_launch failed with code {rc}')
                return
            arr = launches.native()
            failed = ctypes.c_int32(-1)
# ... 16 lines not shown
```

transfusion_pytorch_amd/params.py:

```python
from __future__ import annotations

import math
from dataclasses import dataclass

import numpy as np
import torch
from torch import nn

from . import capi


def pad_to(x: int, m: int) -> int:
    return (x + m - 1) // m * m


@dataclass
class ModelDims:
    num_text_tokens: int
    dim: int
    depth: int
    heads: int
    dim_head: int
    dim_latents: tuple
    ff_expansion_factor: float = 4.
# ... 171 lines not shown
        _attach(root, 'transformer.to_time_cond.0.weights', self.fourier_w, buffer=True)
        self.rot_param = nn.Parameter(self.rot_freqs, requires_grad=False)
        _attach(root, 'rotary_emb.freqs', self.rot_param)
        self.shadows = {}
        self._shadow_version = None
        self._epoch = 0
        self._maps = {}
        self._jobs, self._job_table = [], None
        self._exp_ptrs = None
        self.device = torch.device('cpu')

    def view(self, name):
        o, shape = self.offsets[name]
        return self.flat[o:o + int(np.prod(shape))].view(shape)

    def grad_view(self, name):
        o, shape = self.offsets[name]
        return self.grad[o:o + int(np.prod(shape))].view(shape)

    def grad_ptr(self, name, elem_offset=0):
        return self.grad.data_ptr() + 4 * (self.offsets[name][0] + elem_offset)

    def ptr(self, name, elem_offset=0):
        return self.flat.data_ptr() + 4 * (self.offsets[name][0] + elem_offset)

    def reflatten(self, device):
        flat = torch.zeros(self.numel, device=device)
        with torch.no_grad():
            for name, shape in self.specs:
                o = self.offsets[name][0]
                v = flat[o:o + int(np.prod(shape))].view(shape)
                v.copy_(self.params[name].data)
                self.params[name].data = v
                self.params[name].grad = None
        self.flat = flat
        self.grad = torch.zeros(self.numel, device=device) if device.type == 'cuda' else None
        self.device = device
        self.shadows = {}
        self._shadow_version = None
        self._maps = {}

    def mark_dirty(self):
        self._shadow_version = None
        self._epoch += 1

    def params_version(self):
        ver = self.fourier_w._version + (self._epoch << 32)
        base = self.flat.data_ptr()
        exp = self._exp_ptrs
        if exp is None or exp[0] != base:
            exp = self._exp_ptrs = (base, [(name, prm, base + 4 * self.offsets[name][0]) for name, prm in self.params.items()])
        for name, prm, want in exp[1]:
            if prm.data_ptr() != want:
                v = self.view(name)
                if prm.shape != v.shape:
                    raise ValueError(f'parameter {name} was re-assigned with shape {tuple(prm.shape)}, the model was built for {tuple(v.shape)}')
                with torch.no_grad():
                    v.copy_(prm.data)
                prm.data = v
                self._shadow_version = None
            ver += prm._version
        return ver

    def ensure_grad_views(self):
        fresh = [n for n, p in self.params.items() if p.grad is None]
        if len(fresh) == len(self.params):
            self.grad.zero_()
        else:
            for n in fresh:
                self.grad_view(n).zero_()
        for n in fresh:
            self.params[n].grad = self.grad_view(n)

    def _map(self, key, arr):
        if key not in self._maps:
            self._maps[key] = torch.from_numpy(np.ascontiguousarray(arr, dtype=np.int32)).to(self.device)
        return self._maps[key]

    def _shadow(self, key, rows, cols):
        if key not in self.shadows:
            self.shadows[key] = torch.zeros(rows, cols, device=self.device, dtype=torch.bfloat16)
        return self.shadows[key]

    def _cast(self, stream, src_ptr, ld_src, Rs, Cs, dst, rowmap=None, transpose=False, n_rows_logical=None):
        ld_dst, Rd = dst.shape[1], dst.shape[0]
        assert ld_dst % 8 == 0
        nb = ((ld_dst + 63) // 64) * ((Rd + 63) // 64) if transpose else (Rd * ld_dst + 2047) // 2048
        self._jobs.append((dict(src=src_ptr, ld_src=ld_src, Rs=Rs, Cs=Cs, rowmap=capi.ptr(rowmap), dst=dst.data_ptr(), ld_dst=ld_dst, Rd=Rd,
                                Cd=n_rows_logical if transpose else ld_dst, transposed=int(transpose)), nb))

    def _launch_casts(self, stream):
        key = (self.flat.data_ptr(), len(self._jobs))
        if self._job_table is None or self._job_table[0] != key:
            J = capi.STRUCTS['tfx_cast_job']
            arr = (J * len(self._jobs))()
            first = 0
            for i, (f, nb) in enumerate(self._jobs):
                for k, v in f.items():
                    setattr(arr[i], k, v)
                arr[i].first_block = first
                first += nb
            import ctypes
            raw = torch.frombuffer(bytearray(ctypes.string_at(ctypes.addressof(arr), ctypes.sizeof(arr))), dtype=torch.uint8)
            self._job_table = (key, raw.to(self.device), len(self._jobs), first)
        _, tab, nj, nblk = self._job_table
        capi.check(capi.lib().tfx_cast_batch(tab.data_ptr(), nj, nblk, stream), 'tfx_cast_batch')

    def refresh_shadows(self, stream, force=False):
        ver = self.params_version()
        if not force and ver == self._shadow_version:
            return
        md = self.md
        d, hd, di, dip, D = md.dim, md.hd, md.di, md.dip, md.depth
        S, C = self._shadow, self._cast
        self._jobs = []
        C(stream, self.ptr('transformer.layers.0.1.to_film.weight'), 4 * d, md.nt3, 4 * d, S('ada', md.nt3, 4 * d))
        C(stream, self.ptr('transformer.layers.0.1.to_film.weight'), 4 * d, md.nt3, 4 * d, S('ada_t', 4 * d, md.nt3), transpose=True, n_rows_logical=md.nt3)
        C(stream, self.ptr('transformer.to_time_cond.1.weight'), d + 1, 4 * d, d + 1, S('time', 4 * d, md.kf))
        gmap = self._map('geglu', geglu_phys_to_ref_rows(di, dip))
        dh = md.dim_head
        if dh != 64:
            qmap = self._map('heads', head_phys_to_ref_rows(md.heads, dh))
            gam_map = self._map('gamma', np.where(np.arange(64) < dh, np.arange(64), -1))
        for i in range(D):
            p = f'transformer.layers.{i}'
            if md.has_skip(i):
                C(stream, self.ptr(f'{p}.0.weight'), 2 * d, d, 2 * d, S(f'skip{i}', d, 2 * d))
                C(stream, self.ptr(f'{p}.0.weight'), 2 * d, d, 2 * d, S(f'skip_t{i}', 2 * d, d), transpose=True, n_rows_logical=d)
            if dh == 64:
                C(stream, self.ptr(f'{p}.1.fn.to_qk.0.weight'), d, md.nq, d, S(f'qkvg{i}', md.nq, d))
                C(stream, self.ptr(f'{p}.1.fn.to_qk.0.weight'), d, md.nq, d, S(f'qkvg_t{i}', d, md.ldq), transpose=True, n_rows_logical=md.nq)
                C(stream, self.ptr(f'{p}.1.fn.to_out.1.weight'), hd, d, hd, S(f'out{i}', d, hd))
                C(stream, self.ptr(f'{p}.1.fn.to_out.1.weight'), hd, d, hd, S(f'out_t{i}', hd, d), transpose=True, n_rows_logical=d)
            else:
                hdk = md.hdk
                C(stream, self.ptr(f'{p}.1.fn.to_qk.0.weight'), d, md.nq, d, S(f'qkvg{i}', md.nqk, d), rowmap=qmap)
                C(stream, self.ptr(f'{p}.1.fn.to_qk.0.weight'), d, md.nq, d, S(f'qkvg_t{i}', d, md.ldq), rowmap=qmap, transpose=True, n_rows_logical=md.nqk)
                wo = self.ptr(f'{p}.1.fn.to_out.1.weight')
                C(stream, wo, dh, d * md.heads, dh, S(f'out{i}', d, hdk).view(d * md.heads, 64))
                ot = S(f'out_t{i}', hdk, d)
                for h in range(md.heads):
                    C(stream, wo + 4 * h * dh, hd, d, dh, ot[h * 64:(h + 1) * 64], transpose=True, n_rows_logical=d)
                for nm in ('q', 'k'):
                    key = f'g{nm}{i}'
                    if key not in self.shadows:
                        self.shadows[key] = torch.zeros(64, device=self.device)
                    capi.check(capi.lib().tfx_gather_f32(self.ptr(f'{p}.1.fn.{nm}_norm.gamma'), gam_map.data_ptr(), self.shadows[key].data_ptr(), 64, stream), 'gather_f32')
            C(stream, self.ptr(f'{p}.2.fn.net.0.weight'), d, 2 * di, d, S(f'ff1{i}', 2 * dip, d), rowmap=gmap)
            C(stream, self.ptr(f'{p}.2.fn.net.0.weight'), d, 2 * di, d, S(f'ff1_t{i}', d, 2 * dip), rowmap=gmap, transpose=True, n_rows_logical=2 * dip)
            C(stream, self.ptr(f'{p}.2.fn.net.3.weight'), di, d, di, S(f'ff2{i}', d, dip))
            C(stream, self.ptr(f'{p}.2.fn.net.3.weight'), di, d, di, S(f'ff2_t{i}', dip, d), transpose=True, n_rows_logical=d)
            b1 = self.shadows.get(f'ff1b{i}')
            if b1 is None:
                b1 = self.shadows[f'ff1b{i}'] = torch.zeros(2 * dip, device=self.device)
            capi.check(capi.lib().tfx_gather_f32(self.ptr(f'{p}.2.fn.net.0.bias'), gmap.data_ptr(), b1.data_ptr(), 2 * dip, stream), 'gather_f32')
        if (md.pos_types or md.ext_types) and 'eye' not in self.shadows:
            self.shadows['eye'] = torch.eye(d, device=self.device, dtype=torch.bfloat16)
        for t, dl in enumerate(md.dim_latents):
            dlp = pad_to(dl, 64)
            if t in md.ext_types:
                continue
            if dl != d:
                C(stream, self.ptr(f'latent_to_model_projs.{t}.weight'), dl, d, dl, S(f'in{t}', d, dlp))
            C(stream, self.ptr(f'model_to_latent_projs.{t}.weight'), d, dl, d, S(f'outp{t}', dl, d))
            C(stream, self.ptr(f'model_to_latent_projs.{t}.weight'), d, dl, d, S(f'outp_t{t}', d, dlp), transpose=True, n_rows_logical=dl)
        C(stream, self.ptr('text_embed.weight'), d, md.vocab, d, S('embed', md.vocab, d))
        C(stream, self.ptr('to_text_logits.weight'), d, md.vocab, d, S('logits', md.vp, d))
        C(stream, self.ptr('to_text_logits.weight'), d, md.vocab, d, S('logits_t', d, md.vp), transpose=True, n_rows_logical=md.vocab)
        self._launch_casts(stream)
        self._shadow_version = ver
```

transfusion_pytorch_amd/transfusion.py:

```python
from __future__ import annotations

import contextlib
import ctypes
import os
from typing import NamedTuple

import numpy as np
import torch
from torch import nn

from . import capi
from .engine import Plan
from .ode import check_odeint_kwargs
from .packing import fast_signature, is_int_tensor, scan_batch, scan_signature, token_maps, token_segments
from .axial import ContinuousAxialPositionalEmbedding
from .params import ModelDims, ParamStore


class LossBreakdown(NamedTuple):
    total: torch.Tensor
    text: torch.Tensor
    flow: list
    velocity: list | None = None
    recon: list | None = None
# ... 528 lines not shown
    def _rope_tables(self, max_pos: int):
        if self._rope is None or self._rope[0].shape[0] <= max_pos:
            P = max(2048, 1 << (max_pos + 1).bit_length())
            freqs = self.store.rot_param.detach().float().cpu()
            ang = torch.arange(P, dtype=torch.float32)[:, None] * freqs[None, :]
            cos, sin = torch.ones(P, 32), torch.zeros(P, 32)
            cos[:, :freqs.numel()] = ang.cos(); sin[:, :freqs.numel()] = ang.sin()
            self._rope = (cos.to(self.device).contiguous(), sin.to(self.device).contiguous())
        return self._rope

    def _plan(self, b, n, I, R, training):
        dp_groups = getattr(self, '_dp_groups', 0) if training else 0
        key = (b, n, I, tuple(sorted(R.items())), training, dp_groups)
        plan = self._plans.pop(key, None)
        if plan is None:
            while len(self._plans) >= 8:
                self._plans.pop(next(iter(self._plans)))
            plan = Plan(self.store, b, n, I, R, training=training, dp_groups=dp_groups)
            budget = float(os.environ.get('TFX_PLAN_BUDGET_GB', 0)) * 2 ** 30 or 0.4 * torch.cuda.get_device_properties(self.device).total_memory
            while self._plans and sum(p.nbytes for p in self._plans.values()) + plan.nbytes > budget:
                self._plans.pop(next(iter(self._plans)))
        self._plans[key] = plan
        return plan

    def _structure(self, key, build):
        S = self._struct_cache.pop(key, None)
        if S is None:
            while len(self._struct_cache) >= 32:
                self._struct_cache.pop(next(iter(self._struct_cache)))
            S = build()
        self._struct_cache[key] = S
        return S

    def _build_structure(self, modalities, return_loss, add_meta=True, pad_n=1, presig=None):
        dev = self.device
        if presig is not None:
            P = scan_signature(*presig, num_modalities=self.num_modalities, dim_latents=self.dim_latents, sos_id=self.sos_id, eos_id=self.eos_id,
                               meta_id=self.meta_id, som_ids=self.som_ids, eom_ids=self.eom_ids, add_sos_eos=return_loss, add_meta=add_meta)
        else:
            P = self._scan(modalities, add_sos_eos=return_loss, add_meta=add_meta)
        b = P.b
        n = P.n_full - 1 if return_loss else P.n_full
        n_true = n
        if pad_n > 1 and n % pad_n:
            n = (n + pad_n - 1) // pad_n * pad_n
            n_new = n + 1 if return_loss else n
            old = P.n_full
            th = np.full((b, n_new), -1, dtype=np.int32); th[:, :old] = P.text_host; P.text_host = th
            cd = np.zeros((b, n_new), dtype=bool); cd[:, :old] = P.cfg_droppable; P.cfg_droppable = cd
            P.text_dest = (P.text_dest // old) * n_new + (P.text_dest % old)
            for t in P.row_pos:
                rp = P.row_pos[t].astype(np.int64)
                P.row_pos[t] = ((rp // old) * n_new + (rp % old)).astype(np.int32)
            P.n_full = n_new
        tm = token_maps(P, n, self.num_modalities)
        seg_start, seg_len = token_segments(tm.tok_inst, balance=True)
        R = {t: int(len(v)) for t, v in P.row_inst.items()}
        num_mod = np.bincount(P.inst_b, minlength=b)
        host = dict(text_host=P.text_host, text_dest=P.text_dest, cfg_droppable=P.cfg_droppable, tok_inst=tm.tok_inst, kv_end=tm.kv_end, q_start=tm.q_start,
                    rot_pos=tm.rot_pos, inst_b=P.inst_b, inst_m=P.inst_m, seg_start=seg_start, seg_len=seg_len, num_mod=num_mod)
        for t in R:
            rp = P.row_pos[t].astype(np.int64)
            rb, rl = rp // P.n_full, rp % P.n_full
            host[('row_tok', t)] = np.where(rl < n, rb * n + rl, -1)
            host[('row_inst', t)] = P.row_inst[t]
        offs, pos = {}, 0
        for k, a in host.items():
            offs[k] = (pos, a.size, a.shape); pos += (a.size + 3) // 4 * 4
        arena = torch.empty(max(pos, 4), dtype=torch.int32, pin_memory=(dev.type == 'cuda'))
        av = arena.numpy()
        for k, a in host.items():
            o, sz, _ = offs[k]
            av[o:o + sz] = np.asarray(a).reshape(-1)
        darena = arena.to(dev, non_blocking=True)
        D = lambda k: darena[offs[k][0]:offs[k][0] + offs[k][1]].view(offs[k][2])
        tok_inst = D('tok_inst')
        S = dict(P=P, tm=tm, b=b, n=n, n_true=n_true, I=len(P.inst_b), R=R, num_mod=num_mod,
                 text_host=D('text_host'), text_dest=D('text_dest').long(), cfg_droppable=D('cfg_droppable') != 0, tok_inst=tok_inst,
                 kv_end=D('kv_end').reshape(-1), q_start=D('q_start').reshape(-1), rot_pos=D('rot_pos').reshape(-1),
                 is_mod=tok_inst >= 0, minus1=torch.full((b, n), -1, dtype=torch.int32, device=dev),
                 inst_b=D('inst_b').long(), inst_m=D('inst_m').long(), row_tok={t: D(('row_tok', t)) for t in R}, row_inst={t: D(('row_inst', t)) for t in R},
                 seg_start=D('seg_start'), seg_len=D('seg_len'), _arena=(arena, darena))
        S['num_mod_dev'] = D('num_mod').float()
        D = lambda a: torch.from_numpy(np.ascontiguousarray(a)).to(dev)
        if self.has_recon_loss and return_loss:
            n_inst = np.bincount(P.inst_type, minlength=self.num_modalities).astype(np.float64)
            S['recw'] = {t: D((1. / (n_inst[t] * P.inst_len[P.row_inst[t]].astype(np.float64))).astype(np.float32)) for t in R}
        P.user_text, P.latents = None, None
        return S

    def _scan(self, modalities, add_sos_eos, add_meta=True):
        return scan_batch(modalities, num_modalities=self.num_modalities, dim_latents=self.dim_latents, sos_id=self.sos_id, eos_id=self.eos_id,
                          meta_id=self.meta_id, som_ids=self.som_ids, eom_ids=self.eom_ids, add_sos_eos=add_sos_eos, add_meta=add_meta)

    def _forward_plain(self, samples, times, add_meta=False, pad_n=64):
        self._require_gpu()
        dev, stream = self.device, self._stream()
        ext_ctx = None
        if self._ext:
            with torch.no_grad():
                samples, ext_ctx = self._ext_preprocess(samples, None, return_loss=False)
        sig, user_text, latents = fast_signature(samples)
        S = self._structure((sig, 'plain', add_meta, pad_n), lambda: self._build_structure(samples, False, add_meta=add_meta, pad_n=pad_n))
        tm, b, n, I, R = S['tm'], S['b'], S['n'], S['I'], S['R']
        self.store.refresh_shadows(stream)
        Ip = -(-I // 64) * 64 if I > 0 else 0
        Rp = {t: -(-r // 256) * 256 for t, r in R.items()}
        if Ip > 0:
            for t in range(self.num_modalities):
                Rp.setdefault(t, 256)
        plan = self._plan(b, n, Ip, Rp, training=False)
        plan.load_structure(S, self._rope_tables(int(tm.rot_pos.max()) if tm.rot_pos.size else 0), S['tok_inst'], S['kv_end'], S['q_start'], S['rot_pos'],
                            rows={t: (S['row_tok'][t], S['row_inst'][t]) for t in R})
        self._load_text(plan, S, user_text)
        if I > 0:
            plan.inst_time.zero_()
            plan.inst_time[:I].copy_(times.to(dev, torch.float32)[S['inst_b'], S['inst_m']])
        for t in Rp:
            if t in R:
                r = R[t]
                if t in plan.ext:
                    plan.lat[t]['tok'][:r].copy_(torch.cat(ext_ctx[t]['tok']))
                else:
                    plan.lat[t]['x'][:r].copy_(torch.cat(latents[t]).to(dev, torch.float32))
                if t in plan.ext_add:
                    P = S['P']
                    plan.lat[t]['add'][:r].copy_(self._pos_rows(t, [P.inst_shape[g] for g in range(I) if int(P.inst_type[g]) == t]))
            if t not in plan.ext:
                plan.set_noise(t, None)
        Plan.run(plan.fwd, stream, 0, plan.fwd_logits_end)
        return plan, S

    def _default_times(self, num_modalities_host: np.ndarray, nm=None):
        b, m = len(num_modalities_host), int(num_modalities_host.max()) if len(num_modalities_host) else 0
        if m == 0:
            return torch.empty((b, 0), device=self.device)
        if nm is None:
            nm = torch.from_numpy(num_modalities_host.astype(np.float32)).to(self.device)
        rand_num = torch.floor(torch.rand(b, device=self.device) * nm)
        seq = torch.arange(m, device=self.device)
        prev = seq[None, :] < rand_num[:, None]
        cur = torch.rand(b, device=self.device)
        return torch.where(prev, torch.full((), 0.5, device=self.device), cur[:, None].expand(b, m))

    def _resolve_ema(self, ema):
        if ema is not None and hasattr(ema, 'ema_model'):
            ema = ema.ema_model
        if ema is not None and not isinstance(ema, Transfusion):
            raise NotImplementedError('velocity_consistency_ema_model must be a native Transfusion (or the EMA wrapper of one)')
        if ema is self:
            raise ValueError('velocity_consistency_ema_model is the model itself: the teacher pass would overwrite the activations the backward needs - pass an EMA copy (create_ema)')
        return ema

    def forward(self, modalities, times=None, num_modalities_to_times_fn=None, modality_type=None, cache=None, decode_length=None,
                decoding_text_or_modality=None, velocity_consistency_ema_model=None, velocity_consistency_delta_time=1e-3,
                return_only_pred_flows=False, return_loss=True, return_breakdown=False, return_embed=False, return_hiddens=False,
                return_kv_cache=False, return_times=False, prob_uncond=None, _hidden_request=None):
        self._require_gpu()
        from .modality_processing import process_native
        if PROCESSING_STRATEGIES.get(self.modality_processing) is not process_native:
            raise NotImplementedError(f'PROCESSING_STRATEGIES[{self.modality_processing!r}] is not the native packer: Transfusion.forward runs the fused MI355X step, '
                                      'whose packing (host structure scan + tfx_noise_mix + the row-scattered latent_to_model GEMM) is part of its launch list; '
                                      'call a custom strategy directly (it receives the model) or restore the registry entry')
        if torch.is_tensor(modalities):
            if modalities.dtype in (torch.int32, torch.int64):
                return self.forward_text(modalities, return_loss=return_loss, return_embed=return_embed, cache=cache,
# ... 16 lines not shown
                                        return_kv_cache=return_kv_cache, return_hiddens=return_hiddens, return_times=return_times)
        ema = self._resolve_ema(velocity_consistency_ema_model)
        return_loss = (return_loss and not return_embed) or return_only_pred_flows or ema is not None
        dev, stream, md = self.device, self._stream(), self.md
        hreq = _hidden_request or {}
        hid_only = train_hiddens and not torch.is_grad_enabled() and bool(hreq.get('hiddens_only')) and ema is None and not return_only_pred_flows

        ext_ctx = orig_times = None
        packer_in = modalities
        if self._ext:
            if times is None:
                num_mod = np.array([_num_modalities(sample) for sample in modalities], dtype=np.int64)
                fn = num_modalities_to_times_fn
                times = fn(torch.from_numpy(num_mod).to(dev)) if fn is not None else self._default_times(num_mod)
            times = times.to(dev, torch.float32)
            if ema is not None:
                orig_times = times.clone()
                times = times * (1. - velocity_consistency_delta_time)
            modalities, ext_ctx = self._ext_preprocess(modalities, times, return_loss)

        sig, user_text, latents = fast_signature(modalities)
        add_meta = return_loss or not return_embed
        S = self._structure((sig, return_loss, add_meta), lambda: self._build_structure(
            modalities, return_loss, add_meta=add_meta, pad_n=_TRAIN_PAD if return_loss else 1, presig=(sig, user_text, latents)))
        P, I = S['P'], S['I']
        self._live_n_true = S['n_true']

        if times is None:
            fn = num_modalities_to_times_fn
            times = fn(S['num_mod_dev'].long()) if fn is not None else self._default_times(S['num_mod'], S['num_mod_dev'])
        times = times.to(dev, torch.float32)
        if ema is not None and orig_times is None:
            orig_times = times.clone()
            times = times * (1. - velocity_consistency_delta_time)

        self.store.refresh_shadows(stream)
        plan = self._step_plan(S, return_loss, hid_only, no_teacher=ema is None and not return_only_pred_flows)
        if train_hiddens and not hid_only and torch.is_grad_enabled() and not plan.pull:
            raise NotImplementedError('return_hiddens next to the loss (hidden taps) needs the pull-form AttentionResidual backward: depth <= 32 and dim <= 1024 '
                                      '(under torch.no_grad() the hiddens come back without a tap)')

        prob_uncond = self.prob_uncond if prob_uncond is None else prob_uncond
        self._load_text(plan, S, user_text, prob_uncond if self.training else 0., labels=return_loss)
        if I > 0:
            plan.inst_time[:I].copy_(times[S['inst_b'], S['inst_m']])
        rows_in = self._load_latents(plan, S, latents, ext_ctx, return_loss)

        if not return_loss:
            Plan.run(plan.fwd, stream, 0, plan.fwd_embed_end if return_embed else plan.fwd_logits_end)
            if not return_embed:
                return _pack_outputs(self._logits_out(plan), (return_times, times))
            flows = self._pred_flow_closures(P, self._clean_sources(packer_in, times) if md.model_output_clean else None)
            return _pack_outputs((self._embed_out(plan), flows), (return_times, times))
        hid = None
        if train_hiddens:
            hid = (list(range(md.depth + 2)) if return_hiddens is True else sorted({int(k) % (md.depth + 2) for k in return_hiddens}), bool(hreq.get('raw')))
        if hid_only:
            Plan.run(plan.fwd, stream, 0, plan.fwd_embed_end)
            hiddens = self._hiddens_list(hid, self._hiddens_out(plan, S['n_true'], *hid))
            return _pack_outputs(None, (True, hiddens), (return_times, times), (_hidden_request is not None, (plan, S['n_true'])))
        if return_only_pred_flows:
            return self._pred_flows_out(plan, S, ext_ctx)
        def teacher_flows():
            with _teacher_pass(ema, flat_pred_flows=True):
                return ema(velocity_modalities, times=orig_times + velocity_consistency_delta_time, return_only_pred_flows=True)
        loss, breakdown, hid_out = self._losses(plan, S, ext_ctx, rows_in, teacher_flows if ema is not None else None, hid)
        return _pack_outputs(loss, (return_breakdown, breakdown), (train_hiddens, self._hiddens_list(hid, hid_out)), (return_times, times),
                             (_hidden_request is not None, (plan, S['n_true'])))

    def _step_plan(self, S, return_loss, hid_only, no_teacher):
        md, I, R = self.md, S['I'], S['R']
        bucket = (return_loss and no_teacher and not self._ext and not md.pos_types and not self.has_recon_loss
                  and not md.model_output_clean and os.environ.get('TFX_PLAN_BUCKETS', '1') != '0')
        Ip = _bucket(I, 64) if (bucket and I > 0) else I
        Rp = {t: _bucket(r, 256) for t, r in R.items()} if bucket else R
        plan = self._plan(S['b'], S['n'], Ip, Rp, training=return_loss and not hid_only)
        if return_loss and not hid_only:
            plan.clear_taps()
        if md.model_output_clean:
            plan.set_clean_mode('model')
        if plan.loaded_structure is not S:
            tm = S['tm']
            plan.load_structure(S, self._rope_tables(int(tm.rot_pos.max()) if tm.rot_pos.size else 0), S['tok_inst'], S['kv_end'], S['q_start'], S['rot_pos'],
                                segments=(S['seg_start'], S['seg_len']), rows={t: (S['row_tok'][t], S['row_inst'][t]) for t in R}, set_rows=return_loss)
        return plan

    def _load_text(self, plan, S, user_text, prob_uncond=0., labels=False):
        dev, n = self.device, S['n']
        text_full = S['text_host'].clone()
        if user_text:
            text_full.view(-1).index_copy_(0, S['text_dest'], torch.cat(user_text).to(dev, torch.int32))
        if prob_uncond > 0:
            drop_rows = torch.rand(S['b'], device=dev) < prob_uncond
            text_full = text_full.masked_fill(S['cfg_droppable'] & drop_rows[:, None], self.null_text_id)
        plan.text_ids.copy_(text_full[:, :n].reshape(-1))
        if labels:
            lab = text_full[:, 1:]
            lab = torch.where(S['is_mod'] | (lab == self.null_text_id), S['minus1'], lab)
            plan.labels.copy_(lab.reshape(-1))

    def _load_latents(self, plan, S, latents, ext_ctx, return_loss):
        P, I, R = S['P'], S['I'], S['R']
        rows_in = []
        for t in R:
            lt = plan.lat[t]
            if t in plan.ext_add:
                rows = self._pos_rows(t, [P.inst_shape[g] for g in range(I) if int(P.inst_type[g]) == t])
                lt['add'].copy_(rows.detach())
                rows_in.append(('add', t, rows))
            if t in plan.ext:
                rows = torch.cat(ext_ctx[t]['tok']) if len(ext_ctx[t]['tok']) > 1 else ext_ctx[t]['tok'][0]
                lt['tok'].copy_(rows.detach())
                rows_in.append(('tok', t, rows))
                continue
            lt['x'][:R[t]].copy_(torch.cat(latents[t]), non_blocking=True)
            if return_loss:
                self._fill_noise(lt['eps'][:R[t]], t)
            plan.set_noise(t, lt['eps'].data_ptr() if return_loss else None)
        return rows_in

    def _fill_noise(self, eps, t, reshape=False):
        if self._noise_override is None:
            eps.normal_()
        else:
            eps.copy_(self._noise_override[t].reshape(eps.shape) if reshape else self._noise_override[t])

    def _pred_flows_out(self, plan, S, ext_ctx):
        md, P, R = self.md, S['P'], S['R']
        Plan.run(plan.fwd, self._stream(), 0, plan.fwd_pred_end)
        ext_preds = {t: self._ext_decode(t, plan.embed.index_select(0, plan.row_tok[t].long().clamp(min=0)).float(), ext_ctx[t]) for t in R if t in plan.ext}
        if self._flat_pred_flows:
            return {t: (ext_preds[t] if t in plan.ext else plan.lat[t]['pred']) for t in R}
        out = [[] for _ in range(self.num_modalities)]
        cursor = {t: 0 for t in R}
        for gi in range(len(P.inst_b)):
            t, L = int(P.inst_type[gi]), int(P.inst_len[gi])
            if t in plan.ext:
                out[t].append(ext_preds[t][cursor[t]]); cursor[t] += 1
                continue
            rows = plan.lat[t]['pred'][cursor[t]:cursor[t] + L]; cursor[t] += L
            out[t].append(self._from_channel_last(t, rows.view(*P.inst_shape[gi], md.dim_latents[t]).clone()))
        return out

    def _losses(self, plan, S, ext_ctx, rows_in, teacher_flows, hid):
        md, M, stream, acc = self.md, self.num_modalities, self._stream(), plan.acc
        P, tm, R = S['P'], S['tm'], S['R']
        total = float(P.total_tokens)
        w = {t: float(tm.is_type[t]) / total for t in R}
        native = [t for t in sorted(R) if t not in plan.ext]
        den = {t: R[t] * md.dim_latents[t] for t in native}
        plan.set_loss_scales(self.text_loss_weight / total, {t: 2.0 * self.flow_loss_weight * w[t] / den[t] for t in native})
        plan.set_ce_vocab(md.vocab)
        self._bwd_scale = None
        plan.acc.zero_()
        Plan.run(plan.fwd, stream, graph='auto')

        text_loss = acc[0] / acc[1].clamp(min=1.)
        loss = self.text_loss_weight * acc[0] / total
        flow_losses = {}
        for t in native:
            flow_losses[t] = acc[2 + t] / den[t]
            loss = loss + self.flow_loss_weight * flow_losses[t] * w[t]

        velocity_losses = None
        if teacher_flows is not None:
            teacher = teacher_flows()
            velocity_losses = {}
# ... 434 lines not shown

    def _modality_velocity_loss(self, plan, t, ema, teacher_in, teacher_times, flow_ext=None):
        with _teacher_pass(ema):
            teacher = ema.forward_modality(teacher_in, times=teacher_times, modality_type=t, encode_modality=False, return_loss=False)
            if flow_ext is not None:
                return torch.nn.functional.mse_loss(flow_ext, teacher)
            if self.channel_first_latent[t]:
                teacher = teacher.movedim(1, -1)
        lt = plan.lat[t]
        lt['vel'].copy_(teacher.reshape(lt['vel'].shape))
        va = plan._vel_args[t]
        va.pred, va.flow, va.grad_scale = lt['vel'].data_ptr(), lt['flow'].data_ptr(), 0.0
        Plan.run(plan.vel, self._stream())
        return plan.acc[2 + self.num_modalities + t] / lt['vel'].numel()

    def _modality_recon_loss(self, plan, t, x, times, target):
        lt, dec, dl = plan.lat[t], self.modality_decoder[t], self.md.dim_latents[t]
        if dec is None:
            if self.modality_encoder[t] is not None:
                raise ValueError('reconstruction loss with a modality encoder needs the matching modality decoder')
            lt['recw'].fill_(1. / (x.numel() // dl))
            ra = plan._rec_args[t]
            ra.recon_mode, ra.grad_scale = 1, 2.0 * self.reconstruction_loss_weight / dl
            Plan.run(plan.rec, self._stream())
            return plan.acc[2 + 2 * self.num_modalities + t] / dl
        with torch.no_grad():
            tt = times.view(-1, *([1] * (x.ndim - 1)))
            rec = lt['eps'].view(x.shape) + lt['pred'].view(x.shape) * (1. - tt)
            dec.eval()
            return torch.nn.functional.mse_loss(dec(rec.movedim(-1, 1) if self.channel_first_latent[t] else rec), target.float())

    @torch.no_grad()
    def generate_modality_only(self, batch_size=1, modality_type=None, fixed_modality_shape=None, modality_steps=16,
                               return_unprocessed_modalities=False):
        self._require_gpu()
        if self.num_modalities > 1 and modality_type is None:
            raise AssertionError('`modality_type` must be explicitly passed in on forward when training on greater than 1 modality')
        t = 0 if modality_type is None else int(modality_type)
        shape = fixed_modality_shape if fixed_modality_shape is not None else self.modality_default_shape[t]
        assert shape is not None
        dev = self.device
        y = self._gen_noise_override.to(dev, torch.float32).clone() if getattr(self, '_gen_noise_override', None) is not None \
            else torch.randn((batch_size, *shape, self.md.dim_latents[t]), device=dev)
        if self.channel_first_latent[t]:
            y = y.movedim(-1, 1).contiguous()
        was_training = self.training
        self.eval()
        try:
            grid = torch.linspace(0., 1., modality_steps, device=dev)
            f = lambda tt, yy: self.forward_modality(yy, times=tt.expand(batch_size), modality_type=t, encode_modality=False, return_loss=False)
            if self.ode_method != 'midpoint':
                from .sampling import _ode_rk_solve
                vel = lambda tt, yy: (f(torch.full((1,), tt, device=dev), yy).float().contiguous(), None)
                y = _ode_rk_solve(self.ode_method, modality_steps, y, vel, 1., self._stream())
            else:
                for i in range(modality_steps - 1):
                    t0, dt = grid[i], grid[i + 1] - grid[i]
                    y_mid = y + f(t0, y) * (dt * 0.5)
                    y = y + dt * f(t0 + dt * 0.5, y_mid)
        finally:
            self.train(was_training)
        if self.modality_decoder[t] is not None:
            self.modality_decoder[t].eval()
            y = self.modality_decoder[t](y)
        return y

    def _native_backward(self, grad_out, step_id):
        plan, live_id = self._live
        if live_id != step_id:
            raise RuntimeError('backward() of a stale loss: the native engine keeps the activations of the latest forward only')
        if self._consumed == step_id:
            raise RuntimeError('backward() through the native Transfusion step a second time: the engine keeps one set of loss seeds per '
                               'forward (call forward again; retain_graph is not supported)')
        self._consumed = step_id
        ps = self.store
        ps.ensure_grad_views()
        go = grad_out.reshape(()).to(torch.float32)
        if self._bwd_scale is not None:
            go = go * self._bwd_scale
        lib, stream = capi.lib(), self._stream()
        sp = ctypes.c_void_p(stream)
        for seed in [plan.dlogits] + [lt['dpred'] for lt in plan.lat.values() if 'dpred' in lt]:
            capi.check(lib.tfx_scale_bf16_dev(seed.data_ptr(), seed.numel(), go.data_ptr(), sp), 'tfx_scale_bf16_dev')
        plan.dtables.zero_()
        if self.md.model_output_clean and plan.clean_mode == 'model' and len(plan.clean_bwd):
            Plan.run(plan.clean_bwd, stream)
        red = getattr(self, '_grad_reducer', None)
        if red is None or red.defer or not plan.bwd_cuts or not (torch.distributed.is_available() and torch.distributed.is_initialized()):
            if red is not None and red.defer:
                red.check_fresh()
            plan.run_bwd(stream)
            return
        red.check_fresh()
        red.begin()
        lo = 0
        for idx, first, last in plan.bwd_cuts:
            plan.run_bwd(stream, lo, idx)
            red.group_ready(first, last)
            lo = idx
        plan.run_bwd(stream, lo, None)

    @torch.no_grad()
    def sample_many(self, prompts=None, max_length=2048, text_temperature=1., text_min_p=0.1, fixed_modality_shape=None,
                    force_modality_at_start=None, init_modality_noise=None, modality_steps=16, return_unprocessed_modalities=False,
                    cfg_scale=3., _pos_emb_in_decode=False):
        from .sampling import Sampler
        was_training = self.training
        self.eval()
        try:
            if self._ext:
                plist = prompts if isinstance(prompts, list) else [prompts]
                outs = [self._sample_one_through_forward(pr, max_length=max_length, text_temperature=text_temperature, text_min_p=text_min_p, cache_kv=False,
                                                         fixed_modality_shape=fixed_modality_shape, force_modality_at_start=force_modality_at_start,
                                                         init_modality_noise=init_modality_noise, modality_steps=modality_steps, cfg_scale=cfg_scale)
                        for pr in plist]
                return outs if return_unprocessed_modalities else self.decode_modalities(outs)
            special = any(self.channel_first_latent) or any(e is not None for e in self.modality_encoder) or any(d is not None for d in self.modality_decoder)
            if special and prompts is not None:
                prompts = [self._normalize_prompt(pr) for pr in (prompts if isinstance(prompts, list) else [prompts])]
            out = Sampler(self).sample_many(prompts, max_length=max_length, text_temperature=text_temperature, text_min_p=text_min_p,
                                            fixed_modality_shape=fixed_modality_shape, force_modality_at_start=force_modality_at_start,
                                            init_modality_noise=init_modality_noise, modality_steps=modality_steps, cfg_scale=cfg_scale,
                                            pos_emb_in_decode=_pos_emb_in_decode)
            if special:
                out = [[(p[0], self._from_channel_last(p[0], p[1])) if isinstance(p, tuple) else p for p in sample] for sample in out]
                if not return_unprocessed_modalities:
                    out = self.decode_modalities(out)
            return out
        finally:
            self.train(was_training)

    def _normalize_prompt(self, pr):
        if pr is None:
            return None
        single = isinstance(pr, tuple) or torch.is_tensor(pr)
        parts = self._encode_modalities([[pr] if single else list(pr)])[0]
        out = []
        for part in parts:
            if torch.is_tensor(part) and part.is_floating_point():
                part = (0, part)
            if isinstance(part, tuple) and self.channel_first_latent[part[0]]:
                part = (part[0], part[1].movedim(0, -1))
            out.append(part)
        return out[0] if single else out

    @torch.no_grad()
    def sample_one(self, prompt=None, max_length=2048, text_temperature=1., text_min_p=0.1, cache_kv=None, fixed_modality_shape=None,
                   force_modality_at_start=None, init_modality_noise=None, modality_steps=16, return_unprocessed_modalities=False, cfg_scale=3.):
        if cache_kv is False and not self._ext and not self.model_output_clean:
            was_training = self.training
            self.eval()
            try:
                out = self._sample_one_through_forward(prompt, max_length=max_length, text_temperature=text_temperature, text_min_p=text_min_p, cache_kv=False,
                                                       fixed_modality_shape=fixed_modality_shape, force_modality_at_start=force_modality_at_start,
                                                       init_modality_noise=init_modality_noise, modality_steps=modality_steps, cfg_scale=cfg_scale)
                return out if return_unprocessed_modalities else self.decode_modalities(out)
            finally:
                self.train(was_training)
        return self.sample_many([prompt], max_length=max_length, text_temperature=text_temperature, text_min_p=text_min_p,
                                fixed_modality_shape=fixed_modality_shape, force_modality_at_start=force_modality_at_start,
                                init_modality_noise=init_modality_noise, modality_steps=modality_steps,
                                return_unprocessed_modalities=return_unprocessed_modalities, cfg_scale=cfg_scale, _pos_emb_in_decode=True)[0]

    sample = sample_one

    @torch.no_grad()
    def _sample_one_through_forward(self, prompt=None, max_length=2048, text_temperature=1., text_min_p=0.1, cache_kv=False, fixed_modality_shape=None,
# ... 136 lines not shown
```

Before: 2538 samples/s.

## Fuse weight-shadow casts, cast+colsum for FiLM grads, gather rows before TN GEMM

Several independent changes. The plain and transposed bf16 weight-shadow casts are merged into one dual-output cast job, and the per-step gather_f32 launches are folded into the batched cast kernel. The dtables cast and the FiLM bias column sum now happen in one kernel. The latent projection weight gradient gathers rows into a dense buffer before the TN GEMM instead of using a rowmapped B operand. Zeroing of dtables is limited to the rows not written by the segments. Together these aim to cut kernel launches and memory passes, at the cost of an extra gather buffer and more complex coverage bookkeeping.

```diff
diff --git a/include/tfx.h b/include/tfx.h
--- a/include/tfx.h
+++ b/include/tfx.h
@@ -269,16 +269,20 @@
 typedef struct { const float* src; int32_t ld_src, Rs, Cs; const int32_t* rowmap; tfx_bf16* dst; int32_t ld_dst, Rd, Cd; } tfx_cast_args;
 int tfx_cast_rows(const tfx_cast_args* a, void* stream);
 int tfx_cast_rows_t(const tfx_cast_args* a, void* stream);
-typedef struct { const float* src; int32_t ld_src, Rs, Cs; const int32_t* rowmap; tfx_bf16* dst; int32_t ld_dst, Rd, Cd; int32_t transposed, first_block; } tfx_cast_job;
+enum { TFX_CAST_PLAIN = 0, TFX_CAST_T = 1, TFX_CAST_DUAL = 2, TFX_CAST_GATHER_F32 = 3 };
+typedef struct { const float* src; int32_t ld_src, Rs, Cs; const int32_t* rowmap; tfx_bf16* dst; int32_t ld_dst, Rd, Cd; int32_t transposed, first_block;
+                 tfx_bf16* dst_t; int32_t ld_dst_t, Rd_t, Cd_t; } tfx_cast_job;
 int tfx_cast_batch(const tfx_cast_job* jobs_dev, int32_t n_jobs, int32_t n_blocks, void* stream);
 int tfx_gather_f32(const float* src, const int32_t* map, float* dst, int32_t n, void* stream);
 int tfx_onehot_bf16(const int32_t* ids, const int32_t* tok_inst, tfx_bf16* out, int32_t T, int32_t ld, void* stream);
 int tfx_scatter_rows_bf16(const tfx_bf16* src, int32_t ld_src, int32_t cols, tfx_bf16* dst, int32_t ld_dst, const int32_t* rowmap, int32_t R, void* stream);
+int tfx_gather_rows_bf16(const tfx_bf16* src, int32_t ld_src, int32_t cols, tfx_bf16* dst, int32_t ld_dst, const int32_t* rowmap, int32_t R, void* stream);
 int tfx_f32_to_bf16(const float* src, tfx_bf16* dst, int64_t n, void* stream);
 int tfx_cast_block_bf16(const float* src, int32_t ld_src, tfx_bf16* dst, int32_t ld_dst, int32_t R, int32_t C, void* stream);
 int tfx_silu_bwd(const tfx_bf16* dy, const tfx_bf16* pre, tfx_bf16* dx, int64_t n, void* stream);
 int tfx_colsum_bf16(const tfx_bf16* src, int32_t ld, int32_t R, int32_t C, const int32_t* colmap, const int32_t* rowmap, float* out, void* stream);
 int tfx_colsum_f32(const float* src, int32_t ld, int32_t R, int32_t C, float* out, void* stream);
+int tfx_cast_block_colsum(const float* src, int32_t ld_src, tfx_bf16* dst, int32_t ld_dst, int32_t R, int32_t C, float* out, void* stream);
 int tfx_add_bf16(const tfx_bf16* a, const tfx_bf16* b, tfx_bf16* out, int64_t n, void* stream);
 int tfx_scale_bf16_dev(tfx_bf16* x, int64_t n, const float* scale, void* stream);
 int tfx_scale_bf16_copy(const tfx_bf16* src, tfx_bf16* dst, int64_t n, float scale, void* stream);
@@ -354,6 +358,7 @@
        TFX_OP_OUTPUT_TO_FLOW = 32, TFX_OP_GATHER_F32 = 33, TFX_OP_ONEHOT_BF16 = 34, TFX_OP_SCATTER_ROWS_BF16 = 35, TFX_OP_F32_TO_BF16 = 36,
        TFX_OP_SILU_BWD = 37, TFX_OP_COLSUM_BF16 = 38, TFX_OP_COLSUM_F32 = 39, TFX_OP_ADD_BF16 = 40, TFX_OP_SCALE_BF16_DEV = 41, TFX_OP_CAST_BLOCK_BF16 = 42, TFX_OP_SCALE_BF16_COPY = 43, TFX_OP_ADALN_POST_PRE_FWD = 44, TFX_OP_LAYER_END_FWD = 45,
        TFX_OP_ATTNRES_PREP = 46, TFX_OP_ATTNRES_PULL_BWD = 47, TFX_OP_ATTNRES_FINISH = 52, TFX_OP_ADALN_PRE_POST_BWD = 53,
+       TFX_OP_CAST_BLOCK_COLSUM = 54, TFX_OP_GATHER_ROWS_BF16 = 55,
        TFX_OP_FORK = 48, TFX_OP_JOIN = 49, TFX_OP_JOIN_RECORD = 50, TFX_OP_JOIN_WAIT = 51 };
 typedef struct { int32_t op; int32_t stream; const void* args; } tfx_launch;
 int tfx_run_list(const tfx_launch* list, int32_t n, void* stream, int32_t* failed_at);
diff --git a/transfusion_pytorch_amd/csrc/runner.hip b/transfusion_pytorch_amd/csrc/runner.hip
--- a/transfusion_pytorch_amd/csrc/runner.hip
+++ b/transfusion_pytorch_amd/csrc/runner.hip
@@ -72,6 +72,11 @@
       return tfx_adaln_pre_post_bwd((const tfx_adaln_pre_args*)r->p0, (const tfx_adaln_post_args*)r->p1, s);
     case TFX_OP_CAST_BLOCK_BF16:
       return tfx_cast_block_bf16((const float*)r->p0, (int32_t)r->i0, (tfx_bf16*)r->p1, (int32_t)r->i1, (int32_t)r->i2, (int32_t)r->i3, s);
+    case TFX_OP_CAST_BLOCK_COLSUM:
+      return tfx_cast_block_colsum((const float*)r->p0, (int32_t)r->i0, (tfx_bf16*)r->p1, (int32_t)r->i1, (int32_t)r->i2, (int32_t)r->i3, (float*)r->p2, s);
+    case TFX_OP_GATHER_ROWS_BF16:
+      return tfx_gather_rows_bf16((const tfx_bf16*)r->p0, (int32_t)r->i0, (int32_t)r->i1, (tfx_bf16*)r->p1, (int32_t)r->i2,
+                                  (const int32_t*)r->p2, (int32_t)r->i3, s);
     case TFX_OP_SCALE_BF16_COPY:
       return tfx_scale_bf16_copy((const tfx_bf16*)r->p0, (tfx_bf16*)r->p1, r->i0, r->f0, s);
     case TFX_OP_SCALE_BF16_DEV:
diff --git a/transfusion_pytorch_amd/csrc/tokenwise.hip b/transfusion_pytorch_amd/csrc/tokenwise.hip
--- a/transfusion_pytorch_amd/csrc/tokenwise.hip
+++ b/transfusion_pytorch_amd/csrc/tokenwise.hip
@@ -1746,6 +1746,60 @@
     }
   }
 }
+TFX_DEV void cast64_dual_body(const tfx_cast_job& j, int bx, int by, float (*tile)[65]) {
+  const int r0 = bx * 64, c0 = by * 64;
+  const int rlog = max(j.Rd, j.Cd_t);
+  {
+    const int cq = threadIdx.x & 15, rr = threadIdx.x >> 4;
+    const int c = c0 + 4 * cq;
+    int rs[4];
+#pragma unroll
+    for (int k = 0; k < 4; k++) {
+      const int r = r0 + rr + 16 * k;
+      rs[k] = r < rlog ? (j.rowmap ? j.rowmap[r] : r) : -1;
+      if (rs[k] >= j.Rs) rs[k] = -1;
+    }
+    f32x4 v[4];
+#pragma unroll
+    for (int k = 0; k < 4; k++) {
+      const f32x4 z = {0.f, 0.f, 0.f, 0.f};
+      v[k] = z;
+      if (rs[k] >= 0 && c < j.Cs) {
+        const float* sp = j.src + (size_t)rs[k] * j.ld_src + c;
+        if (c + 4 <= j.Cs && (((uintptr_t)sp) & 15) == 0) v[k] = *(const f32x4*)sp;
+        else {
+#pragma unroll
+          for (int e = 0; e < 4; e++) if (c + e < j.Cs) v[k][e] = sp[e];
+        }
+      }
+    }
+#pragma unroll
+    for (int k = 0; k < 4; k++) {
+      const int r = r0 + rr + 16 * k;
+      if (r < j.Rd && c < j.Cd) {
+        bf16x4 o;
+#pragma unroll
+        for (int e = 0; e < 4; e++) o[e] = f2bf(v[k][e]);
+        *(bf16x4*)(j.dst + (size_t)r * j.ld_dst + c) = o;
+      }
+      const bool live = r < j.Cd_t;
+#pragma unroll
+      for (int e = 0; e < 4; e++) tile[rr + 16 * k][4 * cq + e] = live ? v[k][e] : 0.f;
+    }
+  }
+  __syncthreads();
+#pragma unroll
+  for (int k = 0; k < 2; k++) {
+    const int q = threadIdx.x + 256 * k, row = q >> 3, ch = q & 7;
+    const int c = c0 + row, r = r0 + 8 * ch;
+    if (c < j.Rd_t && r < j.ld_dst_t) {
+      bf16x8 o;
+#pragma unroll
+      for (int e = 0; e < 8; e++) o[e] = f2bf(tile[8 * ch + e][row]);
+      *(bf16x8*)(j.dst_t + (size_t)c * j.ld_dst_t + r) = o;
+    }
+  }
+}
 __global__ __launch_bounds__(256) void cast_batch_k(const tfx_cast_job* jobs, int n_jobs) {
   __shared__ float tile[64][65];
   int lo = 0, hi = n_jobs - 1;
@@ -1753,7 +1807,12 @@
   const tfx_cast_job j = jobs[lo];
   const tfx_cast_args p = {j.src, j.ld_src, j.Rs, j.Cs, j.rowmap, j.dst, j.ld_dst, j.Rd, j.Cd};
   const int lb = blockIdx.x - j.first_block;
-  if (j.transposed) { const int tx = (p.ld_dst + 63) / 64; cast64_t_body(p, lb % tx, lb / tx, tile); }
+  if (j.transposed == TFX_CAST_DUAL) { const int tx = (max(j.Rd, j.ld_dst_t) + 63) / 64; cast64_dual_body(j, lb % tx, lb / tx, tile); }
+  else if (j.transposed == TFX_CAST_GATHER_F32) {
+    const int i = lb * 256 + threadIdx.x;
+    if (i < j.Rd) { const int m = j.rowmap[i]; ((float*)j.dst)[i] = m >= 0 && m < j.Rs ? j.src[m] : 0.f; }
+  }
+  else if (j.transposed) { const int tx = (p.ld_dst + 63) / 64; cast64_t_body(p, lb % tx, lb / tx, tile); }
   else cast8_body(p, lb);
 }
 __global__ void onehot_k(const int* ids, const int* tok_inst, bf16* out, int T, int ld) {
@@ -1773,6 +1832,20 @@
   const int r = (int)(i / cpr), c = (int)(i % cpr) * 8;
   const int ro = rowmap[r];
   if (ro >= 0) *(bf16x8*)(dst + (size_t)ro * ld_dst + c) = *(const bf16x8*)(src + (size_t)r * ld_src + c);
+}
+__global__ void gather_rows_k(const bf16* src, int ld_src, int cols, bf16* dst, int ld_dst, const int* rowmap, int R) {
+  const long long i = (long long)blockIdx.x * blockDim.x + threadIdx.x;
+  const int cpr = cols / 8;
+  if (i >= (long long)R * cpr) return;
+  const int r = (int)(i / cpr), c = (int)(i % cpr) * 8;
+  const int rs = rowmap[r];
+  bf16x8 o;
+  if (rs >= 0) o = *(const bf16x8*)(src + (size_t)rs * ld_src + c);
+  else {
+#pragma unroll
+    for (int e = 0; e < 8; e++) o[e] = f2bf(0.f);
+  }
+  *(bf16x8*)(dst + (size_t)r * ld_dst + c) = o;
 }
 __global__ void gather_f32_k(const float* src, const int* map, float* dst, int n) {
   int i = blockIdx.x * blockDim.x + threadIdx.x;
@@ -1827,6 +1900,55 @@
     float v = s[0][cx] + s[1][cx] + s[2][cx] + s[3][cx];
     int co = colmap ? colmap[c] : c;
     if (co >= 0 && v != 0.f) atomicAdd(out + co, v);
+  }
+}
+
+__global__ __launch_bounds__(256) void cast_block_colsum_k(const float* src, int ld_src, bf16* dst, int ld_dst, int R, int C, float* out, int rows_per_block) {
+  __shared__ float s[8][32][9];
+  const int cx = threadIdx.x & 31, ry = threadIdx.x >> 5;
+  const int c0 = (blockIdx.x * 32 + cx) * 8;
+  const int rbeg = blockIdx.y * rows_per_block, rend = min(R, rbeg + rows_per_block);
+  float a[8];
+#pragma unroll
+  for (int e = 0; e < 8; e++) a[e] = 0.f;
+  if (c0 < C) {
+    int r = rbeg + ry;
+    for (; r + 24 < rend; r += 32) {
+      f32x4 v[4][2];
+#pragma unroll
+      for (int u = 0; u < 4; u++) {
+        const float* sp = src + (size_t)(r + 8 * u) * ld_src + c0;
+        v[u][0] = *(const f32x4*)sp; v[u][1] = *(const f32x4*)(sp + 4);
+      }
+#pragma unroll
+      for (int u = 0; u < 4; u++) {
+        bf16x8 o;
+#pragma unroll
+        for (int e = 0; e < 4; e++) { o[e] = f2bf(v[u][0][e]); o[4 + e] = f2bf(v[u][1][e]); a[e] += v[u][0][e]; a[4 + e] += v[u][1][e]; }
+        *(bf16x8*)(dst + (size_t)(r + 8 * u) * ld_dst + c0) = o;
+      }
+    }
+    for (; r < rend; r += 8) {
+      const float* sp = src + (size_t)r * ld_src + c0;
+      const f32x4 v0 = *(const f32x4*)sp, v1 = *(const f32x4*)(sp + 4);
+      bf16x8 o;
+#pragma unroll
+      for (int e = 0; e < 4; e++) { o[e] = f2bf(v0[e]); o[4 + e] = f2bf(v1[e]); a[e] += v0[e]; a[4 + e] += v1[e]; }
+      *(bf16x8*)(dst + (size_t)r * ld_dst + c0) = o;
+    }
+  }
+#pragma unroll
+  for (int e = 0; e < 8; e++) s[ry][cx][e] = a[e];
+  __syncthreads();
+  {
+    const int cc = threadIdx.x >> 3, e = threadIdx.x & 7;
+    const int col = (blockIdx.x * 32 + cc) * 8 + e;
+    if (col < C) {
+      float v = 0.f;
+#pragma unroll
+      for (int y = 0; y < 8; y++) v += s[y][cc][e];
+      if (v != 0.f) atomicAdd(out + col, v);
+    }
   }
 }
 
@@ -2256,6 +2378,12 @@
   long long n = (long long)R * (cols / 8);
   hipLaunchKernelGGL(scatter_rows_k, dim3((unsigned)((n + 255) / 256)), dim3(256), 0, ST(s), src, ld_src, cols, dst, ld_dst, rowmap, R); RET();
 }
+int tfx_gather_rows_bf16(const tfx_bf16* src, int32_t ld_src, int32_t cols, tfx_bf16* dst, int32_t ld_dst, const int32_t* rowmap, int32_t R, void* s) {
+  if (R == 0 || cols == 0) return 0; if (cols % 8 || ld_src % 8 || ld_dst % 8 || ((uintptr_t)src | (uintptr_t)dst) & 15) return -1;
+  if (!src || !dst || !rowmap) return -2;
+  long long n = (long long)R * (cols / 8);
+  hipLaunchKernelGGL(gather_rows_k, dim3((unsigned)((n + 255) / 256)), dim3(256), 0, ST(s), src, ld_src, cols, dst, ld_dst, rowmap, R); RET();
+}
 int tfx_gather_f32(const float* src, const int32_t* map, float* dst, int32_t n, void* s) {
   if (n == 0) return 0; hipLaunchKernelGGL(gather_f32_k, dim3((n + 255) / 256), dim3(256), 0, ST(s), src, map, dst, n); RET();
 }
@@ -2289,6 +2417,13 @@
   if (R == 0 || C == 0) return 0;
   int rpb = colsum_rows_per_block(R);
   hipLaunchKernelGGL(colsum_k<float>, dim3((C + 63) / 64, (R + rpb - 1) / rpb), dim3(256), 0, ST(s), src, ld, R, C, (const int*)nullptr, (const int*)nullptr, out, rpb); RET();
+}
+int tfx_cast_block_colsum(const float* src, int32_t ld_src, tfx_bf16* dst, int32_t ld_dst, int32_t R, int32_t C, float* out, void* s) {
+  if (C % 8 || ld_src % 8 || ld_dst % 8 || ((uintptr_t)src & 31) || ((uintptr_t)dst & 15)) return -1;
+  if (R == 0 || C == 0) return 0;
+  if (!src || !dst || !out) return -2;
+  int rpb = (R + 63) / 64; rpb = rpb < 8 ? 8 : (rpb + 7) / 8 * 8;
+  hipLaunchKernelGGL(cast_block_colsum_k, dim3((C + 255) / 256, (R + rpb - 1) / rpb), dim3(256), 0, ST(s), src, ld_src, dst, ld_dst, R, C, out, rpb); RET();
 }
 int tfx_sumsq(const float* g, int64_t n, float* out, void* s) {
   if (n == 0) return 0;
diff --git a/transfusion_pytorch_amd/engine.py b/transfusion_pytorch_amd/engine.py
--- a/transfusion_pytorch_amd/engine.py
+++ b/transfusion_pytorch_amd/engine.py
@@ -246,6 +246,7 @@
         self.noise_args = {}
         self.loaded_structure = None
         self._seg_args = []
+        self.n_seg, self.inst_cover = 0, None
         self.seg_start = z(max(T, 1), dtype=torch.int32); self.seg_len = z(max(T, 1), dtype=torch.int32)
         self.pull = training and D <= 32 and md.dim <= 1024
         if self.pull:
@@ -282,6 +283,19 @@
         a = capi.make_args('tfx_gemm_tn_args', M=M, N=N, K=K, splits=splits, accumulate=1, alpha=1.0, **kw)
         a._algo_flops = 2.0 * M * (algo_n or N) * kw['k_valid']
         lst.append(Side(('tfx_gemm_tn', a)) if side else ('tfx_gemm_tn', a))
+
+    def _tn_mapped(self, lst, M, N, K, which, rowmap, **kw):
+        X, ld = kw[which.upper()], kw['ld' + which]
+        dense = dict(kw); dense.setdefault('k_valid', K)
+        probe = capi.make_args('tfx_gemm_tn_args', M=M, N=N, K=K, splits=0, accumulate=1, alpha=1.0, **dense)
+        out = [ctypes.c_int32() for _ in range(4)]
+        if M == 0 or ld != self.md.dim or capi.lib().tfx_gemm_tn_plan(ctypes.byref(probe), *[ctypes.byref(o) for o in out]) != 0 or out[0].value < 0:
+            return self._tn(lst, M, N, K, **kw, **{which + '_rowmap': rowmap})
+        if getattr(self, 'gat', None) is None:
+            self.gat = torch.empty(max(self.R.values()), self.md.dim, device=self.ps.device, dtype=BF16); self.nbytes += self.gat.numel() * 2
+        self._raw(lst, capi.lib().tfx_gather_rows_bf16, X.data_ptr() if hasattr(X, 'data_ptr') else X, ld, self.md.dim, self.gat.data_ptr(), self.md.dim, rowmap.data_ptr(), M)
+        kw[which.upper()] = self.gat
+        self._tn(lst, M, N, K, **kw)
 
     def _tn_group(self, lst, M, problems, side=False):
         if len(problems) < 2 or os.environ.get('TFX_TN_GROUP', '1') == '0':
@@ -587,6 +601,7 @@
 
     def set_segments(self, seg_start, seg_len):
         n_seg = int(seg_start.numel())
+        self.n_seg = n_seg
         self.seg_start[:n_seg].copy_(seg_start); self.seg_len[:n_seg].copy_(seg_len)
         for a in self._seg_args:
             a.n_seg = n_seg
@@ -610,11 +625,23 @@
             if self.row_gat is not self.row_tok:
                 torch.clamp(self.row_tok[t], min=0, out=self.row_gat[t])
 
-    def load_structure(self, S, rope, tok_inst, kv_end, q_start, rot_pos, segments=None, rows=None, set_rows=False):
+    def zero_table_grads(self):
+        c = self.inst_cover
+        if c is None or self.n_seg <= 0 or self.md.dim > 1024:
+            self.dtables.zero_()
+            return
+        n_real, holes = c
+        if n_real < self.dtables.shape[0]:
+            self.dtables[n_real:].zero_()
+        if holes is not None:
+            self.dtables.index_fill_(0, holes, 0.)
+
+    def load_structure(self, S, rope, tok_inst, kv_end, q_start, rot_pos, segments=None, rows=None, set_rows=False, inst_cover=None):
         self.set_rope_tables(*rope)
         self.tok_inst.copy_(tok_inst.view(-1)); self.kv_end.copy_(kv_end); self.q_start.copy_(q_start); self.rot_pos.copy_(rot_pos)
         if segments is not None:
             self.set_segments(*segments)
+        self.inst_cover = inst_cover
         if rows is not None:
             for t, cap in self.R.items():
                 row_tok, row_inst = rows.get(t, (None, None))
@@ -674,8 +701,8 @@
                 continue
             self._nt(L, algo_k=dl, A=lt['dpred'], lda=dlp, B=S[f'outp_t{t}'], ldb=dlp, M=r, N=d, K=dlp, epi=E['TFX_EPI_RESID'], C=self.dembed, ldc=d,
                      R=self.dembed, ldr=d, resid_mapped=1, rowmap=self.row_tok[t])
-            self._tn(L, r, dl, d, A=lt['dpred'], lda=dlp, a_cols=dlp, B=self.embed, ldb=d, b_cols=d, b_rowmap=self.row_gat[t],
-                     C=gp(f'model_to_latent_projs.{t}.weight'), ldc=d)
+            self._tn_mapped(L, r, dl, d, 'b', self.row_gat[t], A=lt['dpred'], lda=dlp, a_cols=dlp, B=self.embed, ldb=d, b_cols=d,
+                            C=gp(f'model_to_latent_projs.{t}.weight'), ldc=d)
         self.tap_final = len(L)
         self._k(L, 'tfx_rmsnorm_bwd', 'tfx_rmsnorm_args', T=T, d=d, x=self.xres[D], gamma=pp('transformer.norm.gamma'), dy=self.dembed,
                 dx=self.gfin, dgamma=gp('transformer.norm.gamma'))
@@ -804,10 +831,9 @@
                 hi = min(i + per, D)
                 off, cols = i * 2 * 3 * d, (hi - i) * 2 * 3 * d
                 w_item = lambda it: L.append(Side(it) if side else it)
-                w_item((lib.tfx_cast_block_bf16, (self.dtables.data_ptr() + 4 * off, nt3, self.dtab_bf.data_ptr() + 2 * off, nt3, I, cols)))
+                w_item((lib.tfx_cast_block_colsum, (self.dtables.data_ptr() + 4 * off, nt3, self.dtab_bf.data_ptr() + 2 * off, nt3, I, cols, gp(f'{p}.1.to_film.bias'))))
                 self._tn(L, I, cols, 4 * d, side=side, A=self.dtab_bf.data_ptr() + 2 * off, lda=nt3, a_cols=cols, B=self.cond, ldb=4 * d, b_cols=4 * d,
                          C=gp(f'{p}.1.to_film.weight'), ldc=4 * d)
-                w_item((lib.tfx_colsum_f32, (self.dtables.data_ptr() + 4 * off, nt3, I, cols, gp(f'{p}.1.to_film.bias'))))
             sync('tfx_join_record', i)
             if self.dp_groups > 0:
                 if i % per == 0:
@@ -845,8 +871,8 @@
             dl = md.dim_latents[t]; dlp = pad_to(dl, 64); lt = self.lat[t]
             if dl == d or t in self.ext:
                 continue
-            self._tn(L, r, d, dl, A=dx0, lda=d, a_cols=d, a_rowmap=self.row_gat[t], B=lt['xt'], ldb=dlp, b_cols=dlp,
-                     C=gp(f'latent_to_model_projs.{t}.weight'), ldc=dl)
+            self._tn_mapped(L, r, d, dl, 'a', self.row_gat[t], A=dx0, lda=d, a_cols=d, B=lt['xt'], ldb=dlp, b_cols=dlp,
+                            C=gp(f'latent_to_model_projs.{t}.weight'), ldc=dl)
             cs = [dx0.data_ptr(), d, int(self.noise_args[t].R), d, None, self.row_tok[t].data_ptr(), gp(f'latent_to_model_projs.{t}.bias')]
             self._rows_dep[t].append((cs, 2))
             L.append((lib.tfx_colsum_bf16, cs))
diff --git a/transfusion_pytorch_amd/params.py b/transfusion_pytorch_amd/params.py
--- a/transfusion_pytorch_amd/params.py
+++ b/transfusion_pytorch_amd/params.py
@@ -277,12 +277,25 @@
             self.shadows[key] = torch.zeros(rows, cols, device=self.device, dtype=torch.bfloat16)
         return self.shadows[key]
 
-    def _cast(self, stream, src_ptr, ld_src, Rs, Cs, dst, rowmap=None, transpose=False, n_rows_logical=None):
+    def _cast(self, stream, src_ptr, ld_src, Rs, Cs, dst, rowmap=None):
         ld_dst, Rd = dst.shape[1], dst.shape[0]
         assert ld_dst % 8 == 0
-        nb = ((ld_dst + 63) // 64) * ((Rd + 63) // 64) if transpose else (Rd * ld_dst + 2047) // 2048
         self._jobs.append((dict(src=src_ptr, ld_src=ld_src, Rs=Rs, Cs=Cs, rowmap=capi.ptr(rowmap), dst=dst.data_ptr(), ld_dst=ld_dst, Rd=Rd,
-                                Cd=n_rows_logical if transpose else ld_dst, transposed=int(transpose)), nb))
+                                Cd=ld_dst, transposed=capi.ENUMS['TFX_CAST_PLAIN']), (Rd * ld_dst + 2047) // 2048))
+
+    def _cast2(self, src_ptr, ld_src, Rs, Cs, dst, dst_t, rowmap=None, n_rows_logical=None):
+        ld_dst, (Rd, Cd) = dst.stride(0), dst.shape
+        ld_t, Rd_t = dst_t.stride(0), dst_t.shape[0]
+        assert ld_dst % 8 == 0 and Cd % 8 == 0 and ld_t % 8 == 0 and dst_t.shape[1] == ld_t
+        nb = ((max(Rd, ld_t) + 63) // 64) * ((max(Cd, Rd_t) + 63) // 64)
+        self._jobs.append((dict(src=src_ptr, ld_src=ld_src, Rs=Rs, Cs=Cs, rowmap=capi.ptr(rowmap), dst=dst.data_ptr(), ld_dst=ld_dst, Rd=Rd, Cd=Cd,
+                                transposed=capi.ENUMS['TFX_CAST_DUAL'], dst_t=dst_t.data_ptr(), ld_dst_t=ld_t, Rd_t=Rd_t, Cd_t=n_rows_logical), nb))
+
+    def _gather(self, key, src_ptr, n_src, vmap, n):
+        if key not in self.shadows:
+            self.shadows[key] = torch.zeros(n, device=self.device)
+        self._jobs.append((dict(src=src_ptr, ld_src=1, Rs=n_src, Cs=1, rowmap=vmap.data_ptr(), dst=self.shadows[key].data_ptr(), ld_dst=n, Rd=n, Cd=n,
+                                transposed=capi.ENUMS['TFX_CAST_GATHER_F32']), (n + 255) // 256))
 
     def _launch_casts(self, stream):
         key = (self.flat.data_ptr(), len(self._jobs))
@@ -307,10 +320,9 @@
             return
         md = self.md
         d, hd, di, dip, D = md.dim, md.hd, md.di, md.dip, md.depth
-        S, C = self._shadow, self._cast
+        S, C, C2 = self._shadow, self._cast, self._cast2
         self._jobs = []
-        C(stream, self.ptr('transformer.layers.0.1.to_film.weight'), 4 * d, md.nt3, 4 * d, S('ada', md.nt3, 4 * d))
-        C(stream, self.ptr('transformer.layers.0.1.to_film.weight'), 4 * d, md.nt3, 4 * d, S('ada_t', 4 * d, md.nt3), transpose=True, n_rows_logical=md.nt3)
+        C2(self.ptr('transformer.layers.0.1.to_film.weight'), 4 * d, md.nt3, 4 * d, S('ada', md.nt3, 4 * d), S('ada_t', 4 * d, md.nt3), n_rows_logical=md.nt3)
         C(stream, self.ptr('transformer.to_time_cond.1.weight'), d + 1, 4 * d, d + 1, S('time', 4 * d, md.kf))
         gmap = self._map('geglu', geglu_phys_to_ref_rows(di, dip))
         dh = md.dim_head
@@ -320,35 +332,22 @@
         for i in range(D):
             p = f'transformer.layers.{i}'
             if md.has_skip(i):
-                C(stream, self.ptr(f'{p}.0.weight'), 2 * d, d, 2 * d, S(f'skip{i}', d, 2 * d))
-                C(stream, self.ptr(f'{p}.0.weight'), 2 * d, d, 2 * d, S(f'skip_t{i}', 2 * d, d), transpose=True, n_rows_logical=d)
+                C2(self.ptr(f'{p}.0.weight'), 2 * d, d, 2 * d, S(f'skip{i}', d, 2 * d), S(f'skip_t{i}', 2 * d, d), n_rows_logical=d)
             if dh == 64:
-                C(stream, self.ptr(f'{p}.1.fn.to_qk.0.weight'), d, md.nq, d, S(f'qkvg{i}', md.nq, d))
-                C(stream, self.ptr(f'{p}.1.fn.to_qk.0.weight'), d, md.nq, d, S(f'qkvg_t{i}', d, md.ldq), transpose=True, n_rows_logical=md.nq)
-                C(stream, self.ptr(f'{p}.1.fn.to_out.1.weight'), hd, d, hd, S(f'out{i}', d, hd))
-                C(stream, self.ptr(f'{p}.1.fn.to_out.1.weight'), hd, d, hd, S(f'out_t{i}', hd, d), transpose=True, n_rows_logical=d)
+                C2(self.ptr(f'{p}.1.fn.to_qk.0.weight'), d, md.nq, d, S(f'qkvg{i}', md.nq, d), S(f'qkvg_t{i}', d, md.ldq), n_rows_logical=md.nq)
+                C2(self.ptr(f'{p}.1.fn.to_out.1.weight'), hd, d, hd, S(f'out{i}', d, hd), S(f'out_t{i}', hd, d), n_rows_logical=d)
             else:
                 hdk = md.hdk
-                C(stream, self.ptr(f'{p}.1.fn.to_qk.0.weight'), d, md.nq, d, S(f'qkvg{i}', md.nqk, d), rowmap=qmap)
-                C(stream, self.ptr(f'{p}.1.fn.to_qk.0.weight'), d, md.nq, d, S(f'qkvg_t{i}', d, md.ldq), rowmap=qmap, transpose=True, n_rows_logical=md.nqk)
+                C2(self.ptr(f'{p}.1.fn.to_qk.0.weight'), d, md.nq, d, S(f'qkvg{i}', md.nqk, d), S(f'qkvg_t{i}', d, md.ldq), rowmap=qmap, n_rows_logical=md.nqk)
                 wo = self.ptr(f'{p}.1.fn.to_out.1.weight')
-                C(stream, wo, dh, d * md.heads, dh, S(f'out{i}', d, hdk).view(d * md.heads, 64))
-                ot = S(f'out_t{i}', hdk, d)
+                o, ot = S(f'out{i}', d, hdk), S(f'out_t{i}', hdk, d)
                 for h in range(md.heads):
-                    C(stream, wo + 4 * h * dh, hd, d, dh, ot[h * 64:(h + 1) * 64], transpose=True, n_rows_logical=d)
+                    C2(wo + 4 * h * dh, hd, d, dh, o[:, h * 64:(h + 1) * 64], ot[h * 64:(h + 1) * 64], n_rows_logical=d)
                 for nm in ('q', 'k'):
-                    key = f'g{nm}{i}'
-                    if key not in self.shadows:
-                        self.shadows[key] = torch.zeros(64, device=self.device)
-                    capi.check(capi.lib().tfx_gather_f32(self.ptr(f'{p}.1.fn.{nm}_norm.gamma'), gam_map.data_ptr(), self.shadows[key].data_ptr(), 64, stream), 'gather_f32')
-            C(stream, self.ptr(f'{p}.2.fn.net.0.weight'), d, 2 * di, d, S(f'ff1{i}', 2 * dip, d), rowmap=gmap)
-            C(stream, self.ptr(f'{p}.2.fn.net.0.weight'), d, 2 * di, d, S(f'ff1_t{i}', d, 2 * dip), rowmap=gmap, transpose=True, n_rows_logical=2 * dip)
-            C(stream, self.ptr(f'{p}.2.fn.net.3.weight'), di, d, di, S(f'ff2{i}', d, dip))
-            C(stream, self.ptr(f'{p}.2.fn.net.3.weight'), di, d, di, S(f'ff2_t{i}', dip, d), transpose=True, n_rows_logical=d)
-            b1 = self.shadows.get(f'ff1b{i}')
-            if b1 is None:
-                b1 = self.shadows[f'ff1b{i}'] = torch.zeros(2 * dip, device=self.device)
-            capi.check(capi.lib().tfx_gather_f32(self.ptr(f'{p}.2.fn.net.0.bias'), gmap.data_ptr(), b1.data_ptr(), 2 * dip, stream), 'gather_f32')
+                    self._gather(f'g{nm}{i}', self.ptr(f'{p}.1.fn.{nm}_norm.gamma'), dh, gam_map, 64)
+            C2(self.ptr(f'{p}.2.fn.net.0.weight'), d, 2 * di, d, S(f'ff1{i}', 2 * dip, d), S(f'ff1_t{i}', d, 2 * dip), rowmap=gmap, n_rows_logical=2 * dip)
+            C2(self.ptr(f'{p}.2.fn.net.3.weight'), di, d, di, S(f'ff2{i}', d, dip), S(f'ff2_t{i}', dip, d), n_rows_logical=d)
+            self._gather(f'ff1b{i}', self.ptr(f'{p}.2.fn.net.0.bias'), 2 * di, gmap, 2 * dip)
         if (md.pos_types or md.ext_types) and 'eye' not in self.shadows:
             self.shadows['eye'] = torch.eye(d, device=self.device, dtype=torch.bfloat16)
         for t, dl in enumerate(md.dim_latents):
@@ -357,10 +356,8 @@
                 continue
             if dl != d:
                 C(stream, self.ptr(f'latent_to_model_projs.{t}.weight'), dl, d, dl, S(f'in{t}', d, dlp))
-            C(stream, self.ptr(f'model_to_latent_projs.{t}.weight'), d, dl, d, S(f'outp{t}', dl, d))
-            C(stream, self.ptr(f'model_to_latent_projs.{t}.weight'), d, dl, d, S(f'outp_t{t}', d, dlp), transpose=True, n_rows_logical=dl)
+            C2(self.ptr(f'model_to_latent_projs.{t}.weight'), d, dl, d, S(f'outp{t}', dl, d), S(f'outp_t{t}', d, dlp), n_rows_logical=dl)
         C(stream, self.ptr('text_embed.weight'), d, md.vocab, d, S('embed', md.vocab, d))
-        C(stream, self.ptr('to_text_logits.weight'), d, md.vocab, d, S('logits', md.vp, d))
-        C(stream, self.ptr('to_text_logits.weight'), d, md.vocab, d, S('logits_t', d, md.vp), transpose=True, n_rows_logical=md.vocab)
+        C2(self.ptr('to_text_logits.weight'), d, md.vocab, d, S('logits', md.vp, d), S('logits_t', d, md.vp), n_rows_logical=md.vocab)
         self._launch_casts(stream)
         self._shadow_version = ver
diff --git a/transfusion_pytorch_amd/transfusion.py b/transfusion_pytorch_amd/transfusion.py
--- a/transfusion_pytorch_amd/transfusion.py
+++ b/transfusion_pytorch_amd/transfusion.py
@@ -634,6 +634,8 @@
                  inst_b=D('inst_b').long(), inst_m=D('inst_m').long(), row_tok={t: D(('row_tok', t)) for t in R}, row_inst={t: D(('row_inst', t)) for t in R},
                  seg_start=D('seg_start'), seg_len=D('seg_len'), _arena=(arena, darena))
         S['num_mod_dev'] = D('num_mod').float()
+        holes = np.setdiff1d(np.arange(len(P.inst_b)), tm.tok_inst[tm.tok_inst >= 0])
+        S['inst_cover'] = (len(P.inst_b), torch.from_numpy(holes.astype(np.int64)).to(dev) if holes.size else None)
         D = lambda a: torch.from_numpy(np.ascontiguousarray(a)).to(dev)
         if self.has_recon_loss and return_loss:
             n_inst = np.bincount(P.inst_type, minlength=self.num_modalities).astype(np.float64)
@@ -816,7 +818,8 @@
         if plan.loaded_structure is not S:
             tm = S['tm']
             plan.load_structure(S, self._rope_tables(int(tm.rot_pos.max()) if tm.rot_pos.size else 0), S['tok_inst'], S['kv_end'], S['q_start'], S['rot_pos'],
-                                segments=(S['seg_start'], S['seg_len']), rows={t: (S['row_tok'][t], S['row_inst'][t]) for t in R}, set_rows=return_loss)
+                                segments=(S['seg_start'], S['seg_len']), rows={t: (S['row_tok'][t], S['row_inst'][t]) for t in R}, set_rows=return_loss,
+                                inst_cover=S['inst_cover'])
         return plan
 
     def _load_text(self, plan, S, user_text, prob_uncond=0., labels=False):
@@ -1417,7 +1420,7 @@
         sp = ctypes.c_void_p(stream)
         for seed in [plan.dlogits] + [lt['dpred'] for lt in plan.lat.values() if 'dpred' in lt]:
             capi.check(lib.tfx_scale_bf16_dev(seed.data_ptr(), seed.numel(), go.data_ptr(), sp), 'tfx_scale_bf16_dev')
-        plan.dtables.zero_()
+        plan.zero_table_grads()
         if self.md.model_output_clean and plan.clean_mode == 'model' and len(plan.clean_bwd):
             Plan.run(plan.clean_bwd, stream)
         red = getattr(self, '_grad_reducer', None)
```

New measurement: 2558 samples/s, median of 6. Within noise of the previous version (+0.8%).
